# mims-harvard/SubGNN

Measured on AMD Instinct MI355X. Metric: subgraphs/sec fwd+bwd (all 3 channels on) + achieved HBM GB/s, higher is better.
Workload: dtype f32; 1 GPU; synthetic DENSITY-style BA base graph n=1000000 m=10 (9998512 undirected edges), 50000 BFS subgraphs x 20 nodes per GPU (weak form; BASELINE configs[3] "50k sharded across 8" as worded is --scaling strong), all_density hparams (N 10/43, P 57/183, S 42, 1 layer), D=64, full pass = sampling + similarities + fwd + bwd + Adam; subgraphs_per_gpu=50000, subgraphs_total=50000

## Files before the change

include/subgnn_hip.h:

```cpp
#ifndef SUBGNN_HIP_H
#define SUBGNN_HIP_H

#include <stdint.h>

#ifdef __cplusplus
extern "C" {
#endif

#define SGNN_OK                  0
#define SGNN_ERR_BAD_ARG        -1
#define SGNN_ERR_SET_TOO_LARGE  -2
#define SGNN_ERR_NNZ_TOO_LARGE  -3
#define SGNN_ERR_LAUNCH         -4
#define SGNN_ERR_UNSUPPORTED_D  -5

#define SGNN_ABI_VERSION 13
int sgnn_abi_version(void);
int sgnn_warm_up(void* stream);
const char* sgnn_last_error(void);

int sgnn_degree_sequence(const int64_t* rowptr, const int32_t* col, int64_t nnz,
                         const int32_t* full_degree, const uint8_t* self_loops,
                         const int64_t* set_ptr, const int32_t* set_nodes, int64_t n_sets,
                         int64_t max_set_size, int sorted,
                         int32_t* out_internal, int32_t* out_external, const int32_t* set_order, void* stream);
int sgnn_degree_sequence_sorted_rows(const int64_t* rowptr, const int32_t* col, const int32_t* col_sorted,
                                     int64_t nnz, const int32_t* full_degree, const uint8_t* self_loops,
                                     const int64_t* set_ptr, const int32_t* set_nodes, int64_t n_sets,
                                     int64_t max_set_size, int sorted, int32_t* out_internal,
                                     int32_t* out_external, const int32_t* set_order, void* stream);
int sgnn_degree_sequence_hub_bitmaps(const int64_t* rowptr, const int32_t* col, const int32_t* col_sorted,
                                     int64_t nnz, const int32_t* full_degree, const uint8_t* self_loops,
                                     const int32_t* hub_index, const uint32_t* hub_bits, int64_t hub_words,
                                     const int32_t* node_info, int info_degree,
                                     const int64_t* set_ptr, const int32_t* set_nodes, int64_t n_sets,
                                     int64_t max_set_size, int sorted, int32_t* out_internal,
                                     int32_t* out_external, const int32_t* set_order, void* stream);
int64_t sgnn_degree_sequence_search_threshold(void);
int64_t sgnn_degree_sequence_huge_workspace_bytes(int64_t total_entries);
int sgnn_degree_sequence_huge(const int64_t* rowptr, const int32_t* col, int64_t nnz, const int32_t* full_degree,
                              const int64_t* set_ptr, const int32_t* set_nodes, int64_t n_sets,
                              int64_t total_entries, int32_t* out_internal, int32_t* out_external,
                              void* workspace, int64_t workspace_bytes, void* stream);

int sgnn_cc_labels(const int64_t* rowptr, const int32_t* col_sorted, int64_t nnz,
                   const int64_t* sub_ptr, const int32_t* sub_nodes, int64_t n_subgraphs,
                   int64_t max_sub_len ,
                   int32_t* out_label, void* stream);
int sgnn_sort_sets(const int64_t* set_ptr, const int32_t* set_nodes, int64_t n_sets, int64_t max_set_size,
                   int32_t* out_nodes, int32_t* out_pos, void* stream);
int sgnn_cc_compact_stats(const int64_t* sub_ptr, const int32_t* sub_nodes, const int32_t* labels,
                          int64_t n_subgraphs, int64_t max_sub_len, int32_t* out_n_components,
                          int32_t* out_longest, void* stream);
int sgnn_cc_compact(const int64_t* sub_ptr, const int32_t* sub_nodes, const int32_t* labels,
                    int64_t n_subgraphs, int64_t max_sub_len, int64_t C, int64_t L, int64_t* out, void* stream);
int64_t sgnn_cc_huge_workspace_bytes(int64_t total_nodes);
int sgnn_cc_labels_huge(const int64_t* rowptr, const int32_t* col, int64_t nnz, const int64_t* sub_ptr,
                        const int32_t* sub_nodes, int64_t n_subgraphs, int64_t total_nodes, int32_t* out_label,
                        void* workspace, int64_t workspace_bytes, void* stream);
int sgnn_cc_compact_huge(const int64_t* sub_ptr, const int32_t* sub_nodes, const int32_t* labels,
                         int64_t n_subgraphs, int64_t total_nodes, int write, int64_t C, int64_t L,
                         int32_t* out_n_components, int32_t* out_longest, int64_t* out, void* workspace,
                         int64_t workspace_bytes, void* stream);

int64_t sgnn_subgraph_properties_workspace_bytes(int64_t total_nodes);
int sgnn_subgraph_properties(const int64_t* rowptr, const int32_t* col_sorted, int64_t nnz, int64_t max_id, int rows_simple,
                             const int64_t* sub_ptr, const int32_t* sub_nodes, int64_t n_sets, int64_t max_len,
                             int64_t total_nodes, int64_t* out_counts, int32_t* out_core, void* workspace,
                             int64_t workspace_bytes, void* stream);

int64_t sgnn_khop_border_workspace_bytes(int64_t max_id, int64_t n_sets, int bitmap_in_lds);
int sgnn_khop_border_bitmap_fits_lds(int64_t max_id);
int sgnn_khop_border(const int64_t* rowptr, const int32_t* col, int64_t nnz, int64_t max_id,
                     const int64_t* set_ptr, const int32_t* set_nodes, int64_t n_sets,
                     int k, int ego_dict_mode,
                     int64_t* out_count, const int64_t* out_ptr, int32_t* out_nodes, uint8_t* out_hop,
                     void* workspace, int64_t workspace_bytes, int bitmap_in_lds, void* stream);
int sgnn_khop_border_arena(const int64_t* rowptr, const int32_t* col, int64_t nnz, int64_t max_id,
                           const int64_t* set_ptr, const int32_t* set_nodes, int64_t n_sets, int k,
                           const int64_t* arena_off, int32_t* arena, int64_t* out_count,
                           void* workspace, int64_t workspace_bytes, int bitmap_in_lds, void* stream);
int64_t sgnn_khop_border_sample_workspace_bytes(int64_t max_id, int64_t n_sets, int k, int rows_sorted, int bitmap_in_lds);
int sgnn_khop_border_sample(const int64_t* rowptr, const int32_t* col, const int32_t* col_sorted, int64_t nnz, int64_t max_id,
                            const int64_t* set_ptr, const int32_t* set_nodes, int64_t n_sets, int k,
                            int64_t n_slots, uint64_t seed, uint64_t stream_id, int64_t item_base,
                            int64_t* out_anchor, uint8_t* out_hop, uint8_t* out_allneg, int64_t* out_count,
                            const int32_t* set_order ,
                            void* workspace, int64_t workspace_bytes, int bitmap_in_lds, void* stream);
int sgnn_khop_sample_finish(int64_t* anchor, const uint8_t* hop, const uint8_t* allneg, const int64_t* counts,
                            const int64_t* width, int64_t n_sets, int64_t n_slots, float* sims, void* stream);
int sgnn_khop1_border_sorted(const int64_t* rowptr, const int32_t* col, const int32_t* col_sorted, int64_t nnz, int64_t max_id,
                             const int64_t* set_ptr, const int32_t* set_nodes, int64_t n_sets,
                             int64_t* out_count, const int64_t* out_ptr , int32_t* out_ids ,
                             void* workspace, int64_t workspace_bytes, int bitmap_in_lds, void* stream);

int sgnn_first_occurrence_mask(const int64_t* ids, int64_t n_rows, int64_t row_len, uint8_t* keep, void* stream);
int sgnn_filter_sets(const int64_t* set_ptr, const int32_t* set_nodes, const uint8_t* flags, int64_t n_sets, int64_t* counts,
                     const int64_t* out_ptr, int32_t* out_nodes, void* stream);
int sgnn_pack_rows_count(const int64_t* ids, const uint8_t* mask, int64_t n_rows, int64_t row_len, int64_t* counts,
                         void* stream);
int sgnn_pack_rows_write(const int64_t* ids, const uint8_t* mask, int64_t n_rows, int64_t row_len, const int64_t* ptr,
                         int32_t* nodes, void* stream);
int64_t sgnn_pack_fused_max_rows(void);
int64_t sgnn_pack_fused_max_entries(void);
int sgnn_pack_rows_fused(const int64_t* ids, const uint8_t* mask, int mode, int64_t n_rows, int64_t row_len, int64_t* ptr,
                         int32_t* nodes, void* stream);
int sgnn_filter_sets_fused(const int64_t* set_ptr, const int32_t* set_nodes, const uint8_t* flags, int64_t n_sets,
                           int64_t arena_entries, int64_t* out_ptr, int32_t* out_nodes, void* stream);

int sgnn_sample_anchors_padded(const int64_t* ids, int64_t n_rows, int64_t L, int64_t n_slots,
                               uint64_t seed, uint64_t stream_id, int64_t* out, void* stream);
int sgnn_sample_anchors_ragged(const int64_t* set_ptr, const int32_t* set_nodes, int64_t n_sets,
                               const uint8_t* row_has_pad, int64_t n_slots,
                               uint64_t seed, uint64_t stream_id, int64_t item_base, int64_t* out, void* stream);
int sgnn_sample_border_anchors(const int64_t* ptr, const int32_t* ids, const int64_t* counts, int64_t n_sets,
                               const int64_t* width, int64_t n_slots, uint64_t seed, uint64_t stream_id, int64_t item_base,
                               int hop, int64_t* out_anchor, float* out_sims, void* stream);

int sgnn_choice_ragged(const int64_t* ptr, const int32_t* seq, int64_t n_items, int64_t n_draws,
                       uint64_t seed, uint64_t stream_id, int64_t item_base, int64_t* out, void* stream);

int sgnn_set_keys(const int64_t* set_ptr, const int32_t* set_nodes, int64_t n_sets, uint64_t* out_keys, void* stream);
int sgnn_sample_anchors_ragged_keyed(const int64_t* set_ptr, const int32_t* set_nodes, int64_t n_sets,
                                     const uint8_t* row_has_pad, const uint64_t* keys, int64_t n_slots,
                                     uint64_t seed, uint64_t stream_id, int64_t* out, void* stream);
int sgnn_choice_ragged_keyed(const int64_t* ptr, const int32_t* seq, int64_t n_items, const uint64_t* keys, int64_t n_draws,
                             uint64_t seed, uint64_t stream_id, int64_t* out, void* stream);
int sgnn_sample_border_anchors_keyed(const int64_t* ptr, const int32_t* ids, const uint8_t* hops, int64_t n_sets,
                                     const uint8_t* row_has_pad, const uint64_t* keys, int64_t n_slots, uint64_t seed,
                                     uint64_t stream_id, int64_t* out_anchor, float* out_sims, void* stream);

#define SGNN_OCC_NODE 0
#define SGNN_OCC_COMPONENT 1
int64_t sgnn_occlusion_lds_max(void);
int64_t sgnn_occlusion_workspace_bytes(int64_t total_entries);
int sgnn_occlusion_count(const int64_t* set_ptr, const int32_t* set_nodes, int64_t n_sets, int64_t max_set_len, int mode,
                         const int32_t* labels, int64_t* out_units, int64_t* out_variants, int64_t* out_len,
                         int64_t total_entries, void* workspace, int64_t workspace_bytes, void* stream);
int sgnn_occlusion_write(const int64_t* set_ptr, const int32_t* set_nodes, int64_t n_sets, int64_t max_set_len, int mode,
                         const int32_t* labels, const int64_t* var_ptr, const int64_t* len_scan, int64_t n_variants,
                         int64_t* out_ptr, int32_t* out_nodes, int32_t* out_parent, int32_t* out_unit, uint64_t* out_keys,
                         int64_t total_entries, void* workspace, int64_t workspace_bytes, void* stream);

int sgnn_insertion_count(const int64_t* set_ptr, const int32_t* set_nodes, int64_t n_sets, int64_t max_set_len,
                         const int64_t* cand_ptr, const int32_t* cand_ids, int shared, int64_t* out_variants, void* stream);
int sgnn_insertion_write(const int64_t* set_ptr, const int32_t* set_nodes, int64_t n_sets, int64_t max_set_len,
                         const int64_t* cand_ptr, const int32_t* cand_ids, int shared, const int64_t* var_ptr,
                         const int64_t* entry_ptr, int64_t n_variants, int64_t* out_ptr, int32_t* out_nodes,
                         int32_t* out_parent, int32_t* out_cand, uint64_t* out_keys, void* stream);

int64_t sgnn_seeded_walk_max_size(void);
int sgnn_seeded_walk_sets(const int64_t* rowptr, const int32_t* col, int64_t max_id, const int32_t* seeds, int64_t n_seeds,
                          const int32_t* sizes, int64_t per_seed, int64_t width, uint64_t restart_thr, int64_t max_steps,
                          uint64_t seed, uint64_t stream, int64_t item_base, const int64_t* item_ids, int64_t n_items,
                          int32_t* out_nodes, int32_t* out_len, int32_t* out_steps, uint64_t* out_keys, void* stream_handle);

int sgnn_triangular_walks(const int64_t* rowptr, const int32_t* col, const int32_t* col_sorted, int64_t nnz,
                          const int32_t* node_order, int64_t n_nodes,
                          const int64_t* patch_ptr, const int32_t* patch_nodes,
                          const int64_t* inb_ptr, const int32_t* inb_nodes,
                          int mode, int64_t n_items, int64_t walks_per_patch, int64_t walk_len, double beta,
                          uint64_t seed, uint64_t stream_id, int64_t item_base, int64_t max_id, int kernel, int64_t* out,
                          void* stream);
int sgnn_triangular_walks_both(const int64_t* rowptr, const int32_t* col, const int32_t* col_sorted, int64_t nnz,
                               const int64_t* patch_ptr, const int32_t* patch_nodes, const int64_t* inb_ptr,
                               const int32_t* inb_nodes, int64_t n_items, int64_t walks_per_patch, int64_t walk_len,
                               double beta, uint64_t seed, uint64_t stream_id_int, uint64_t stream_id_bor,
                               int64_t item_base, int64_t max_id, int64_t* out, void* stream);
int sgnn_triangular_walks_variants(void);
int sgnn_triangular_walks_rule(int64_t n_walks, int64_t max_id);
int sgnn_triangular_walks_lists(const int64_t* rowptr, const int32_t* col, const int32_t* col_sorted, int64_t nnz,
                                const int32_t* hub_index, const uint32_t* hub_bits, int64_t hub_words,
                                const int32_t* node_order, int64_t n_nodes,
                                const int64_t* patch_ptr, const int32_t* patch_nodes,
                                const int64_t* inb_ptr, const int32_t* inb_nodes,
                                int mode, int64_t n_items, int64_t walks_per_patch, int64_t walk_len, double beta,
                                uint64_t seed, uint64_t stream_id, int64_t item_base, int64_t max_id, int kernel, int variant,
                                int64_t* out, void* stream);
int sgnn_triangular_walks_both_lists(const int64_t* rowptr, const int32_t* col, const int32_t* col_sorted, int64_t nnz,
                                     const int32_t* hub_index, const uint32_t* hub_bits, int64_t hub_words,
                                     const int64_t* patch_ptr, const int32_t* patch_nodes, const int64_t* inb_ptr,
                                     const int32_t* inb_nodes, int64_t n_items, int64_t walks_per_patch, int64_t walk_len,
                                     double beta, uint64_t seed, uint64_t stream_id_int, uint64_t stream_id_bor,
                                     int64_t item_base, int64_t max_id, int variant, int64_t* out, void* stream);

int sgnn_patch_in_border(const int64_t* rowptr, const int32_t* col, int64_t nnz,
                         const int32_t* node_order, const int32_t* node_pos, int64_t n_nodes,
                         const int64_t* patch_ptr, const int32_t* patch_nodes, int64_t n_patches,
                         uint8_t* out_flag, void* stream);
int64_t sgnn_patch_in_border_huge_workspace_bytes(int64_t total_nodes);
int sgnn_patch_in_border_huge(const int64_t* rowptr, const int32_t* col, int64_t nnz,
                              const int32_t* node_order, const int32_t* node_pos, int64_t n_nodes,
                              const int64_t* patch_ptr, const int32_t* patch_nodes, int64_t n_patches,
                              int64_t total_nodes, uint8_t* out_flag, void* workspace, int64_t workspace_bytes,
                              void* stream);

int sgnn_sp_similarity_dense(const double* apsp, int64_t n_cols,
                             const int64_t* set_ptr, const int32_t* set_nodes, int64_t n_sets,
                             float* out, void* stream);
int64_t sgnn_bfs_hops_workspace_bytes(int64_t max_id, int64_t n_sources, int max_hops);
int sgnn_bfs_hops(const int64_t* rowptr, const int32_t* col, int64_t nnz, int64_t max_id,
                  const int32_t* sources, int64_t n_sources, int max_hops, int node_major, int pull_alpha,
                  uint8_t* dist, void* workspace, int64_t workspace_bytes, void* stream);
int sgnn_min_hops_to_sets(const uint8_t* dist, int64_t n_sources, int64_t max_id, int node_major,
                          const int64_t* set_ptr, const int32_t* set_nodes, int64_t n_sets,
                          float* out, void* stream);
int64_t sgnn_bfs_min_hops_workspace_bytes(int64_t max_id, int64_t n_sources, int max_hops, int64_t n_sets);
int sgnn_bfs_min_hops_to_sets(const int64_t* rowptr, const int32_t* col, int64_t nnz, int64_t max_id,
                              const int32_t* sources, int64_t n_sources, int max_hops, int pull_alpha, int push_levels,
                              const int64_t* set_ptr, const int32_t* set_nodes, int64_t n_sets,
                              float* out, int32_t* out_status, void* workspace, int64_t workspace_bytes, void* stream);
int64_t sgnn_graph_component_labels_workspace_bytes(int64_t max_id);
int sgnn_graph_component_labels(const int64_t* rowptr, const int32_t* col, int64_t nnz, int64_t max_id,
                                int32_t* labels, void* workspace, int64_t workspace_bytes, void* stream);
int64_t sgnn_bfs_min_hops_closing_workspace_bytes(int64_t max_id, int64_t n_sources, int max_hops, int64_t n_sets);
int sgnn_bfs_min_hops_to_sets_closing(const int64_t* rowptr, const int32_t* col, int64_t nnz, int64_t max_id,
                                      const int32_t* sources, int64_t n_sources, int max_hops, int pull_alpha, int push_levels,
                                      const int32_t* labels, const int64_t* set_ptr, const int32_t* set_nodes,
                                      int64_t n_sets, float* out, int32_t* out_status, void* workspace, int64_t workspace_bytes,
                                      void* stream);

int sgnn_dtw_order_keys(const int64_t* x_ptr, const int32_t* x_val, int64_t n_x, int64_t* out_keys, void* stream);
int64_t sgnn_dtw_workspace_bytes(int64_t n_x, int64_t max_x_len, int64_t n_y, int64_t max_y_len);
int sgnn_dtw_similarity(const int64_t* x_ptr, const int32_t* x_val, int64_t n_x, int64_t max_x_len,
                        const int64_t* y_ptr, const int32_t* y_val, int64_t n_y, int64_t max_y_len,
                        int tie_order, int kernel, const int32_t* x_order, float* out, void* workspace,
                        int64_t workspace_bytes, void* stream);
int sgnn_dtw_similarity_live(const int64_t* x_ptr, const int32_t* x_val, int64_t n_x, int64_t max_x_len,
                             const int64_t* y_ptr, const int32_t* y_val, int64_t n_y, int64_t max_y_len,
                             int tie_order, int kernel, const int32_t* x_order, const int64_t* x_live_range, float* out,
                             void* workspace, int64_t workspace_bytes, void* stream);
int64_t sgnn_dtw_rows_bytes(int64_t n_x, int64_t max_x_len);
int64_t sgnn_dtw_rows_header_words(void);
int64_t sgnn_dtw_rows_workspace_bytes(int64_t n_x, int64_t max_x_len, int64_t n_y, int64_t max_y_len);
int sgnn_dtw_prepare_rows(const int64_t* x_ptr, const int32_t* x_val, int64_t n_x, int64_t max_x_len, int kernel,
                          const int32_t* x_order, void* rows, int64_t rows_bytes, int64_t* header, void* stream);
int sgnn_dtw_similarity_rows(const int64_t* rows_header, int64_t n_x, int64_t max_x_len,
                             const int64_t* y_ptr, const int32_t* y_val, int64_t n_y, int64_t max_y_len,
                             int tie_order, int kernel, const int32_t* x_order, float* out, void* workspace,
                             int64_t workspace_bytes, void* stream);
int sgnn_dtw_similarity_rows_live(const int64_t* rows_header, int64_t n_x, int64_t max_x_len,
                                  const int64_t* y_ptr, const int32_t* y_val, int64_t n_y, int64_t max_y_len,
                                  int tie_order, int kernel, const int32_t* x_order, const int64_t* x_live_range, float* out,
                                  void* workspace, int64_t workspace_bytes, void* stream);

int64_t sgnn_dtw_exact_workspace_bytes(int64_t n_x, int64_t max_x_len, int64_t n_y, int64_t max_y_len);
int sgnn_dtw_exact_similarity(const int64_t* x_ptr, const int32_t* x_val, int64_t n_x, int64_t max_x_len,
                              const int64_t* y_ptr, const int32_t* y_val, int64_t n_y, int64_t max_y_len,
                              int kernel, const int32_t* x_order, float* out, void* workspace,
                              int64_t workspace_bytes, void* stream);
int sgnn_dtw_exact_similarity_live(const int64_t* x_ptr, const int32_t* x_val, int64_t n_x, int64_t max_x_len,
                                   const int64_t* y_ptr, const int32_t* y_val, int64_t n_y, int64_t max_y_len,
                                   int kernel, const int32_t* x_order, const int64_t* x_live_range, float* out,
                                   void* workspace, int64_t workspace_bytes, void* stream);
int64_t sgnn_dtwx_rows_bytes(int64_t n_x, int64_t max_x_len);
int64_t sgnn_dtwx_rows_workspace_bytes(int64_t n_x, int64_t max_x_len, int64_t n_y, int64_t max_y_len);
int sgnn_dtwx_prepare_rows(const int64_t* x_ptr, const int32_t* x_val, int64_t n_x, int64_t max_x_len, int kernel,
                                const int32_t* x_order, void* rows, int64_t rows_bytes, int64_t* header, void* stream);
int sgnn_dtwx_similarity_rows(const int64_t* rows_header, int64_t n_x, int64_t max_x_len,
                                   const int64_t* y_ptr, const int32_t* y_val, int64_t n_y, int64_t max_y_len,
                                   int kernel, const int32_t* x_order, float* out, void* workspace,
                                   int64_t workspace_bytes, void* stream);
int sgnn_dtwx_similarity_rows_live(const int64_t* rows_header, int64_t n_x, int64_t max_x_len,
                                        const int64_t* y_ptr, const int32_t* y_val, int64_t n_y, int64_t max_y_len,
                                        int kernel, const int32_t* x_order, const int64_t* x_live_range, float* out,
                                        void* workspace, int64_t workspace_bytes, void* stream);

#define SGNN_TOPK_DOT    0
#define SGNN_TOPK_COSINE 1
#define SGNN_TOPK_L2     2
int64_t sgnn_topk_max_k(void);
int64_t sgnn_topk_rows_workspace_bytes(int64_t Q, int64_t N, int64_t k, int64_t splits);
int sgnn_topk_rows(const float* q, int64_t q_stride, int64_t Q, const float* bank, int64_t b_stride, int64_t N,
                   int64_t D, int64_t k, int metric, const float* q_aux, const float* b_aux, const int64_t* exclude,
                   int64_t splits, float* out_score, int64_t* out_index, void* workspace, int64_t workspace_bytes,
                   void* stream);

int64_t sgnn_kmeans_max_k(void);
int64_t sgnn_kmeans_slots(int64_t N, int64_t K, int64_t D);
int64_t sgnn_kmeans_workspace_bytes(int64_t N, int64_t K, int64_t D);
int sgnn_kmeans_step(const float* x, int64_t x_stride, int64_t N, const float* c, int64_t c_stride, int64_t K, int64_t D,
                     int metric, const float* x_aux, const float* c_aux, const int32_t* prev_assign, int32_t* assign,
                     float* score, void* workspace, int64_t workspace_bytes, void* stream);
int sgnn_kmeans_finish(const void* workspace, int64_t workspace_bytes, int64_t N, int64_t K, int64_t D, int metric,
                       const float* c, int64_t c_stride, float* sums, int32_t* counts, double* inertia, int32_t* empty,
                       float* c_next, float* c_aux_next, int32_t* changed, int64_t it, void* stream);

int sgnn_cc_embed_fwd(const float* E, int64_t D,
                      const int64_t* set_ptr, const int32_t* set_nodes, int64_t n_sets,
                      int aggregator, int64_t padded_len, float* out, int32_t* out_arg, void* stream);
int sgnn_cc_embed_fwd_f16(const uint16_t* E_half, int64_t D,
                          const int64_t* set_ptr, const int32_t* set_nodes, int64_t n_sets,
                          int aggregator, int64_t padded_len, float* out, int32_t* out_arg, void* stream);
int sgnn_cc_embed_bwd(const float* grad_out, int64_t D,
                      const int64_t* set_ptr, const int32_t* set_nodes, int64_t n_sets,
                      int aggregator, const int32_t* arg, float* grad_E, void* stream);

#define SGNN_SRC_DENSE  0
#define SGNN_SRC_GATHER 1
#define SGNN_SRC_SHARED 2

typedef struct sgnn_mpn_args {
    int32_t src;
    int32_t sims_per_edge;
    int64_t R, A, D;
    const float*   x;
    const int64_t* ids;
    int64_t        id_div;
    const uint8_t* edge_mask;
    const uint8_t* row_mask;
    const float*   sims;
    int64_t        sims_ld;
    const int64_t* sim_col;
    const float*   wp;
    const float*   bp;
    int32_t        x_f16;
    const float*   z_act;
    int32_t        flags;
} sgnn_mpn_args;
#define SGNN_MPN_WP_PARTIAL 1
#define SGNN_MPN_RELU_Z     2

int sgnn_mpn_fwd_chunks(const sgnn_mpn_args* args);
int sgnn_mpn_fwd(const sgnn_mpn_args* args, float* agg , float* z , void* stream);
int64_t sgnn_mpn_fwd_many_max_bodies(void);
int sgnn_mpn_fwd_many(int64_t n, const sgnn_mpn_args* args, float* const* agg, float* const* z, void* stream);
int sgnn_mpn_bwd(const sgnn_mpn_args* args, const float* grad_agg, const float* grad_z,
                 float* grad_x, float* grad_wp, void* stream);

int sgnn_attn_scores_epilogue(const float* XU, const float* qW, const float* v, int64_t R, int64_t H,
                              int64_t rows_per_batch, float* out, void* stream);
int64_t sgnn_attn_scores_f16_workspace_bytes(int64_t H);
int sgnn_attn_scores_fwd_f16(const float* X, const float* U, const float* qW, const float* v,
                             int64_t R, int64_t H, int64_t rows_per_batch, float* out,
                             void* workspace, int64_t workspace_bytes, void* stream);

int sgnn_lstm_supported(int64_t hidden_size);
int sgnn_lstm_fwd(const float* pre_x, const float* whh_f, const float* whh_r, const float* bhh_f, const float* bhh_r,
                  int64_t B, int64_t T, int64_t hidden_size, float* y, float* gates, float* cell, float* hprev, void* stream);
int sgnn_lstm_bwd(const float* whh_f, const float* whh_r, const float* gates, const float* cell, const float* dy,
                  int64_t B, int64_t T, int64_t hidden_size, float* dgates, void* stream);

int sgnn_rows_gemm(const float* X, const int64_t* ids, int64_t ldx, int64_t R, int64_t K, const float* W0, const float* W1,
                   const float* b0, const float* b1, int64_t N, float* out, float* x_copy, void* stream);
int sgnn_rows_gemm_nt(const float* A, int64_t R, int64_t K, const float* W0, const float* W1, int64_t N, float* out, void* stream);
int sgnn_lstm_tail_fwd(const float* y, int64_t n_patches, int64_t n_walks, int64_t T, int64_t H2, int last_only,
                       const float* W_lin, const float* b_lin, int64_t D, float* s_out, float* X, void* stream);
int sgnn_lstm_tail_bwd(const float* dX, const float* s, int64_t n_patches, int64_t n_walks, int64_t T, int64_t H2,
                       int last_only, const float* W_lin, int64_t D, float* dy, float* dW_lin, float* db_lin, void* stream);

int sgnn_masked_sum_slot_fwd(const float* x, const uint8_t* mask, int64_t B, int64_t C, int64_t W, float* out,
                             int64_t out_ld, void* stream);
int sgnn_masked_sum_slot_bwd(const float* grad_out, int64_t grad_ld, const uint8_t* mask, int64_t B, int64_t C,
                             int64_t W, float* grad_x, void* stream);
int sgnn_masked_sum_slots_fwd(const float* const* xs, const int64_t* widths, const int64_t* offsets, int64_t n_pieces,
                              const uint8_t* mask, int64_t B, int64_t C, float* out, int64_t out_ld, void* stream);
int sgnn_masked_sum_slots_bwd(const float* grad_out, int64_t grad_ld, const uint8_t* mask, int64_t B, int64_t C,
                              float* const* grad_xs, const int64_t* widths, const int64_t* offsets, int64_t n_pieces, void* stream);

int64_t sgnn_cross_entropy_workspace_bytes(int64_t B);
int sgnn_cross_entropy_fwd(const float* logits, const int64_t* labels, int64_t B, int64_t K, float* lse, float* loss,
                           float* accuracy, void* workspace, int64_t workspace_bytes, void* stream);
int sgnn_cross_entropy_bwd(const float* logits, const int64_t* labels, const float* lse, const float* grad_loss,
                           int64_t B, int64_t K, float* grad_logits, void* stream);

int64_t sgnn_bce_logits_workspace_bytes(int64_t B);
int sgnn_bce_logits_fwd(const float* logits, const int64_t* targets, int64_t B, int64_t K, float* loss, float* accuracy,
                        void* workspace, int64_t workspace_bytes, void* stream);
int sgnn_bce_logits_bwd(const float* logits, const int64_t* targets, const float* grad_loss, int64_t B, int64_t K,
                        float* grad_logits, void* stream);

int sgnn_cross_entropy_fwd_weighted(const float* logits, const int64_t* labels, int64_t B, int64_t K, float* lse, float* loss,
                                    float* accuracy, void* workspace, int64_t workspace_bytes, void* stream,
                                    const float* class_weight);
int sgnn_cross_entropy_bwd_weighted(const float* logits, const int64_t* labels, const float* lse, const float* grad_loss,
                                    int64_t B, int64_t K, float* grad_logits, void* stream, const float* class_weight);
int sgnn_bce_logits_fwd_weighted(const float* logits, const int64_t* targets, int64_t B, int64_t K, float* loss, float* accuracy,
                                 void* workspace, int64_t workspace_bytes, void* stream, const float* weight,
                                 const float* pos_weight);
int sgnn_bce_logits_bwd_weighted(const float* logits, const int64_t* targets, const float* grad_loss, int64_t B, int64_t K,
                                 float* grad_logits, void* stream, const float* weight, const float* pos_weight);

int64_t sgnn_column_sum_workspace_bytes(int64_t R, int64_t A);
int sgnn_column_sum(const float* x, int64_t ld, int64_t R, int64_t A, float* out, void* workspace, int64_t workspace_bytes,
                    void* stream);

int64_t sgnn_readout_many_max(void);
int sgnn_readout_many_fwd(int64_t n, const float* const* sims, const int64_t* sims_ld, const int64_t* const* sim_col,
                          const float* const* X, const float* const* wp, const float* const* bp,
                          const int64_t* const* ids, const uint8_t* const* row_mask, float* const* s, const int64_t* A,
                          const int64_t* off, int64_t D, int64_t B, int64_t C, float* out, int64_t out_ld, void* stream);
int64_t sgnn_readout_many_bwd_workspace_bytes(int64_t n, const int64_t* A, int64_t B, int64_t C);
int sgnn_readout_many_bwd(int64_t n, const float* grad_out, int64_t grad_ld, const float* const* sims, const int64_t* sims_ld,
                          const int64_t* const* sim_col, const float* const* X, const float* const* wp,
                          const float* const* bp, const int64_t* const* ids, const uint8_t* const* row_mask,
                          float* const* s, const int64_t* A, const int64_t* off, int64_t D, int64_t B, int64_t C,
                          float* const* grad_X, float* const* grad_wp, float* const* grad_bp, void* workspace,
                          int64_t workspace_bytes, unsigned* tickets, void* stream);

int64_t sgnn_scatter_add_rows_workspace_bytes(int64_t n_edges, int64_t D);
int64_t sgnn_sort_edges_by_key_workspace_bytes(int64_t n_edges, int64_t max_key);
int sgnn_sort_edges_by_key(const int32_t* keys, int64_t n_edges, int64_t max_key, int32_t* key_sorted, int32_t* order,
                           void* workspace, int64_t workspace_bytes, void* stream);
int sgnn_scatter_add_rows_sorted(const int32_t* order, const int32_t* key_sorted, int64_t n_edges,
                                 const int32_t* edge_row, int64_t edges_per_row,
                                 const float* G, int64_t D, const float* c1, const float* c2, const float* v,
                                 const int32_t* arg, float* table,
                                 void* workspace, int64_t workspace_bytes, void* stream);
int64_t sgnn_scatter_add_rows_multi_workspace_bytes(int64_t total_edges, int64_t D, int64_t max_key);
int sgnn_scatter_add_rows_multi(int64_t n_lists, const int32_t* const* keys, const int64_t* n_edges,
                                const int32_t* const* edge_row, const int64_t* edges_per_row, const float* const* G,
                                const float* const* c1, const float* const* c2, const float* const* v, int64_t D,
                                int64_t max_key, float* table, void* workspace, int64_t workspace_bytes, void* stream);
int64_t sgnn_mpn_bwd_shared_det_workspace_bytes(int64_t R, int64_t A, int64_t D);
int sgnn_mpn_bwd_shared_det(const struct sgnn_mpn_args* args, const float* grad_agg, const float* grad_z,
                            float* grad_x, float* grad_wp, float* grad_bp, void* workspace, int64_t workspace_bytes,
                            void* stream);
int sgnn_mpn_bwd_edges(const struct sgnn_mpn_args* args, const float* grad_z, int32_t* out_keys, float* out_c1,
                       float* out_c2, void* stream);
int sgnn_mpn_bwd_wp_partial(const struct sgnn_mpn_args* args, const float* grad_z, float* partial, int64_t partial_ld,
                            void* stream);
int sgnn_mpn_bwd_edges_many(int64_t n, const struct sgnn_mpn_args* args, const float* const* grad_z, int32_t* const* out_keys,
                            float* const* out_c1, float* const* out_c2, void* stream);

int sgnn_update_fwd(const float* x, const float* aggr, const float* W, const float* b, int64_t R, int64_t D,
                    float* out, void* stream);
int64_t sgnn_update_fwd_chunks_max_rows(void);
int sgnn_update_fwd_chunks(const float* x, const float* aggr_chunks, int64_t n_chunks, const float* W, const float* b,
                           int64_t R, int64_t D, float* out, float* aggr_sum, void* stream);
int64_t sgnn_update_many_max_bodies(void);
int sgnn_update_fwd_many(int64_t n, const float* const* x, const float* const* aggr_chunks, const int64_t* n_chunks,
                         const float* const* W, const float* const* b, int64_t R, int64_t D, float* const* out,
                         float* const* aggr_sum, void* stream);
int sgnn_update_bwd_many(int64_t n, const float* const* grad_out, const float* const* out, const float* const* x,
                         const float* const* aggr, const float* const* W, int64_t R, int64_t D, float* const* grad_x,
                         float* const* grad_aggr, float* const* grad_W, float* const* grad_b, void* workspace,
                         int64_t workspace_bytes, void* stream);
int64_t sgnn_update_bwd_workspace_bytes(int64_t R, int64_t D);
int sgnn_update_bwd(const float* grad_out, const float* out, const float* x, const float* aggr, const float* W,
                    int64_t R, int64_t D, float* grad_x, float* grad_aggr, float* grad_W, float* grad_b,
                    void* workspace, int64_t workspace_bytes, void* stream);

int sgnn_adam_step(float* param, const float* grad, float* exp_avg, float* exp_avg_sq, int64_t n, float lr, float beta1,
                   float beta2, float eps, float weight_decay, int64_t step, const float* grad_scale, void* stream);

int64_t sgnn_optim_partials(const int64_t* numels, int64_t n_tensors);
int sgnn_optim_sumsq(const float* const* grads, const int64_t* numels, int64_t n_tensors, float* partial,
                     int64_t* step_counters, const int64_t* counter_slots, void* stream);
int sgnn_optim_count(int64_t* step_counters, const int64_t* counter_slots, int64_t n_tensors, void* stream);
int sgnn_optim_adam(float* const* params, float* const* grads, float* const* exp_avg, float* const* exp_avg_sq,
                    const int64_t* numels, const int32_t* zero_grad, int64_t n_tensors, float lr, float beta1, float beta2,
                    float eps, const int64_t* steps, const int64_t* step_counters, const int64_t* counter_slots,
                    const int64_t* row_lens, unsigned char* const* row_seen,
                    const float* partial, int64_t n_partial, float max_norm, float* coef_out, void* stream);
int sgnn_optim_adam_lr_table(float* const* params, float* const* grads, float* const* exp_avg, float* const* exp_avg_sq,
                             const int64_t* numels, const int32_t* zero_grad, int64_t n_tensors, const float* lr_table,
                             int64_t lr_len, float beta1, float beta2, float eps, const int64_t* steps,
                             const int64_t* step_counters, const int64_t* counter_slots, const int64_t* row_lens,
                             unsigned char* const* row_seen, const float* partial, int64_t n_partial, float max_norm,
                             float* coef_out, void* stream);


int64_t sgnn_gather_rows_many_max(void);
int sgnn_gather_rows_many(int64_t n, const void* const* src, void* const* dst, const int64_t* row_bytes,
                          const int64_t* src_rows, const int64_t* idx, int64_t B, int32_t* out_of_range, void* stream);

int sgnn_head_supported(int64_t H1, int64_t H2, int64_t K);
int64_t sgnn_head_blocks(int64_t B);
int64_t sgnn_head_partial_floats(int64_t H1, int64_t H2, int64_t K);
int64_t sgnn_head_fwd_workspace_bytes(int64_t B);
int sgnn_head_fwd(const float* z1, int64_t B, int64_t H1, int64_t H2, int64_t K, const float* W2, const float* b2,
                  const float* W3, const float* b3, const int64_t* labels, float p, int64_t* rng, float* a1, float* a2,
                  float* logits, float* lse, float* out, void* workspace, int64_t workspace_bytes, void* stream);
int sgnn_head_bwd(const float* logits, const float* lse, const int64_t* labels, const float* grad_loss,
                  const float* grad_logits, const float* rows, const float* a1, const float* a2, const float* W2,
                  const float* W3, int64_t B, int64_t H1, int64_t H2, int64_t K, float p, float* dz1, float* partial,
                  void* stream);

int sgnn_head_fwd_ml(const float* z1, int64_t B, int64_t H1, int64_t H2, int64_t K, const float* W2, const float* b2,
                     const float* W3, const float* b3, const int64_t* targets, float p, int64_t* rng, float* a1, float* a2,
                     float* logits, float* out, void* workspace, int64_t workspace_bytes, void* stream);
int sgnn_head_bwd_ml(const float* logits, const int64_t* targets, const float* grad_loss, const float* grad_logits,
                     const float* rows, const float* a1, const float* a2, const float* W2, const float* W3, int64_t B,
                     int64_t H1, int64_t H2, int64_t K, float p, float* dz1, float* partial, void* stream);

int sgnn_head_fwd_weighted(const float* z1, int64_t B, int64_t H1, int64_t H2, int64_t K, const float* W2, const float* b2,
                           const float* W3, const float* b3, const int64_t* labels, float p, int64_t* rng, float* a1, float* a2,
                           float* logits, float* lse, float* out, void* workspace, int64_t workspace_bytes, void* stream,
                           const float* class_weight);
int sgnn_head_bwd_weighted(const float* logits, const float* lse, const int64_t* labels, const float* grad_loss,
                           const float* grad_logits, const float* rows, const float* a1, const float* a2, const float* W2,
                           const float* W3, int64_t B, int64_t H1, int64_t H2, int64_t K, float p, float* dz1, float* partial,
                           void* stream, const float* class_weight);
int sgnn_head_fwd_ml_weighted(const float* z1, int64_t B, int64_t H1, int64_t H2, int64_t K, const float* W2, const float* b2,
                              const float* W3, const float* b3, const int64_t* targets, float p, int64_t* rng, float* a1,
                              float* a2, float* logits, float* out, void* workspace, int64_t workspace_bytes, void* stream,
                              const float* weight, const float* pos_weight);
int sgnn_head_bwd_ml_weighted(const float* logits, const int64_t* targets, const float* grad_loss, const float* grad_logits,
                              const float* rows, const float* a1, const float* a2, const float* W2, const float* W3, int64_t B,
                              int64_t H1, int64_t H2, int64_t K, float p, float* dz1, float* partial, void* stream,
                              const float* weight, const float* pos_weight);

int64_t sgnn_contract_rows_max_jobs(void);
int64_t sgnn_contract_rows_blocks(int64_t R, int64_t M, int64_t N);
int sgnn_contract_rows_partial(int64_t n_jobs, const float* const* A, const float* const* B, const int64_t* lda,
                               const int64_t* ldb, const int64_t* M, const int64_t* N, const int64_t* R,
                               float* const* part, float* const* colsum_part, void* stream);
int64_t sgnn_reduce_partials_max_jobs(void);
int sgnn_reduce_partials(int64_t n_jobs, const float* const* part, const int64_t* n_blocks, const int64_t* n,
                         float* const* out, void* stream);

int64_t sgnn_ne_chunk_entries(void);
int sgnn_ne_aggregate(const int64_t* rowptr, const int32_t* col, const float* w, const float* a_self, const float* X,
                      const float* bias, int64_t n_rows, int64_t F, const int32_t* chunk_row, const int64_t* chunk_beg,
                      int64_t n_chunks, const int32_t* long_rows, const int64_t* chunk_first, int64_t n_long,
                      int relu, uint32_t drop_thr, float drop_scale, uint64_t seed, uint64_t stream_id, float* out,
                      float* partial, void* stream);
int sgnn_ne_relu_drop_bwd(const float* grad, const float* out, float* dst, int64_t n, float scale, void* stream);
int sgnn_ne_negatives(const int64_t* rowptr, const int32_t* col_sorted, int64_t n_ids, int64_t n, uint64_t seed,
                      uint64_t stream_id, int64_t item_base, int max_attempts, int32_t* u_out, int32_t* v_out, void* stream);
int64_t sgnn_ne_link_loss_workspace_bytes(void);
int sgnn_ne_link_loss(const float* Z, int64_t F, const int32_t* pu, const int32_t* pv, int64_t n_pairs, int64_t n_pos,
                      float* s_out, float* g_out, float* loss, void* workspace, int64_t workspace_bytes, void* stream);

int sgnn_probe_stream_copy(const void* src, void* dst, int64_t n_bytes, int bytes_per_lane, void* stream);

#ifdef __cplusplus
}
#endif
#endif
```

subgnn_amd/_lib.py:

```python
import ctypes
import os

_HERE = os.path.dirname(os.path.abspath(__file__))
LIB_PATH = os.path.join(_HERE, 'lib', 'libsubgnn_hip.so')

c_i64 = ctypes.c_int64
c_u64 = ctypes.c_uint64
c_int = ctypes.c_int
c_dbl = ctypes.c_double
c_ptr = ctypes.c_void_p


class MpnArgs(ctypes.Structure):
    _fields_ = [('src', ctypes.c_int32), ('sims_per_edge', ctypes.c_int32),
                ('R', c_i64), ('A', c_i64), ('D', c_i64),
                ('x', c_ptr), ('ids', c_ptr), ('id_div', c_i64), ('edge_mask', c_ptr), ('row_mask', c_ptr),
                ('sims', c_ptr), ('sims_ld', c_i64), ('sim_col', c_ptr), ('wp', c_ptr), ('bp', c_ptr),
                ('x_f16', ctypes.c_int32), ('z_act', c_ptr), ('flags', ctypes.c_int32)]


SIGNATURES = {
    'sgnn_abi_version': (c_int, []),
    'sgnn_warm_up': (c_int, [c_ptr]),
    'sgnn_last_error': (ctypes.c_char_p, []),
    'sgnn_degree_sequence': (c_int, [c_ptr, c_ptr, c_i64, c_ptr, c_ptr, c_ptr, c_ptr, c_i64, c_i64, c_int, c_ptr, c_ptr,
                                     c_ptr, c_ptr]),
    'sgnn_degree_sequence_sorted_rows': (c_int, [c_ptr, c_ptr, c_ptr, c_i64, c_ptr, c_ptr, c_ptr, c_ptr, c_i64, c_i64, c_int,
                                                 c_ptr, c_ptr, c_ptr, c_ptr]),
    'sgnn_degree_sequence_hub_bitmaps': (c_int, [c_ptr, c_ptr, c_ptr, c_i64, c_ptr, c_ptr, c_ptr, c_ptr, c_i64, c_ptr, c_int,
                                                 c_ptr, c_ptr, c_i64, c_i64, c_int, c_ptr, c_ptr, c_ptr, c_ptr]),
    'sgnn_degree_sequence_search_threshold': (c_i64, []),
    'sgnn_cc_embed_fwd_f16': (c_int, [c_ptr, c_i64, c_ptr, c_ptr, c_i64, c_int, c_i64, c_ptr, c_ptr, c_ptr]),
    'sgnn_cc_labels': (c_int, [c_ptr, c_ptr, c_i64, c_ptr, c_ptr, c_i64, c_i64, c_ptr, c_ptr]),
    'sgnn_cc_compact_stats': (c_int, [c_ptr, c_ptr, c_ptr, c_i64, c_i64, c_ptr, c_ptr, c_ptr]),
    'sgnn_cc_compact': (c_int, [c_ptr, c_ptr, c_ptr, c_i64, c_i64, c_i64, c_i64, c_ptr, c_ptr]),
    'sgnn_cc_huge_workspace_bytes': (c_i64, [c_i64]),
    'sgnn_degree_sequence_huge_workspace_bytes': (c_i64, [c_i64]),
    'sgnn_degree_sequence_huge': (c_int, [c_ptr, c_ptr, c_i64, c_ptr, c_ptr, c_ptr, c_i64, c_i64, c_ptr, c_ptr, c_ptr, c_i64, c_ptr]),
    'sgnn_cc_labels_huge': (c_int, [c_ptr, c_ptr, c_i64, c_ptr, c_ptr, c_i64, c_i64, c_ptr, c_ptr, c_i64, c_ptr]),
    'sgnn_cc_compact_huge': (c_int, [c_ptr, c_ptr, c_ptr, c_i64, c_i64, c_int, c_i64, c_i64, c_ptr, c_ptr, c_ptr, c_ptr, c_i64, c_ptr]),
    'sgnn_subgraph_properties_workspace_bytes': (c_i64, [c_i64]),
    'sgnn_subgraph_properties': (c_int, [c_ptr, c_ptr, c_i64, c_i64, c_int, c_ptr, c_ptr, c_i64, c_i64, c_i64, c_ptr, c_ptr, c_ptr, c_i64,
                                         c_ptr]),
    'sgnn_patch_in_border_huge_workspace_bytes': (c_i64, [c_i64]),
    'sgnn_patch_in_border_huge': (c_int, [c_ptr, c_ptr, c_i64, c_ptr, c_ptr, c_i64, c_ptr, c_ptr, c_i64, c_i64, c_ptr, c_ptr, c_i64, c_ptr]),
    'sgnn_sort_sets': (c_int, [c_ptr, c_ptr, c_i64, c_i64, c_ptr, c_ptr, c_ptr]),
    'sgnn_khop_border_workspace_bytes': (c_i64, [c_i64, c_i64, c_int]),
    'sgnn_khop_border_bitmap_fits_lds': (c_int, [c_i64]),
    'sgnn_khop_border': (c_int, [c_ptr, c_ptr, c_i64, c_i64, c_ptr, c_ptr, c_i64, c_int, c_int, c_ptr, c_ptr, c_ptr,
                                 c_ptr, c_ptr, c_i64, c_int, c_ptr]),
    'sgnn_khop_border_arena': (c_int, [c_ptr, c_ptr, c_i64, c_i64, c_ptr, c_ptr, c_i64, c_int, c_ptr, c_ptr, c_ptr, c_ptr,
                                       c_i64, c_int, c_ptr]),
    'sgnn_khop_border_sample_workspace_bytes': (c_i64, [c_i64, c_i64, c_int, c_int, c_int]),
    'sgnn_khop_border_sample': (c_int, [c_ptr, c_ptr, c_ptr, c_i64, c_i64, c_ptr, c_ptr, c_i64, c_int, c_i64, c_u64, c_u64, c_i64,
                                        c_ptr, c_ptr, c_ptr, c_ptr, c_ptr, c_ptr, c_i64, c_int, c_ptr]),
    'sgnn_khop1_border_sorted': (c_int, [c_ptr, c_ptr, c_ptr, c_i64, c_i64, c_ptr, c_ptr, c_i64, c_ptr, c_ptr, c_ptr, c_ptr, c_i64,
                                         c_int, c_ptr]),
    'sgnn_sample_border_anchors': (c_int, [c_ptr, c_ptr, c_ptr, c_i64, c_ptr, c_i64, c_u64, c_u64, c_i64, c_int, c_ptr, c_ptr,
                                           c_ptr]),
    'sgnn_sample_anchors_padded': (c_int, [c_ptr, c_i64, c_i64, c_i64, c_u64, c_u64, c_ptr, c_ptr]),
    'sgnn_sample_anchors_ragged': (c_int, [c_ptr, c_ptr, c_i64, c_ptr, c_i64, c_u64, c_u64, c_i64, c_ptr, c_ptr]),
    'sgnn_choice_ragged': (c_int, [c_ptr, c_ptr, c_i64, c_i64, c_u64, c_u64, c_i64, c_ptr, c_ptr]),
    'sgnn_set_keys': (c_int, [c_ptr, c_ptr, c_i64, c_ptr, c_ptr]),
    'sgnn_occlusion_lds_max': (c_i64, []),
    'sgnn_occlusion_workspace_bytes': (c_i64, [c_i64]),
    'sgnn_occlusion_count': (c_int, [c_ptr, c_ptr, c_i64, c_i64, c_int, c_ptr, c_ptr, c_ptr, c_ptr, c_i64, c_ptr, c_i64, c_ptr]),
    'sgnn_occlusion_write': (c_int, [c_ptr, c_ptr, c_i64, c_i64, c_int, c_ptr, c_ptr, c_ptr, c_i64, c_ptr, c_ptr, c_ptr, c_ptr, c_ptr,
                                     c_i64, c_ptr, c_i64, c_ptr]),
    'sgnn_insertion_count': (c_int, [c_ptr, c_ptr, c_i64, c_i64, c_ptr, c_ptr, c_int, c_ptr, c_ptr]),
    'sgnn_insertion_write': (c_int, [c_ptr, c_ptr, c_i64, c_i64, c_ptr, c_ptr, c_int, c_ptr, c_ptr, c_i64, c_ptr, c_ptr, c_ptr, c_ptr,
                                     c_ptr, c_ptr]),
    'sgnn_seeded_walk_max_size': (c_i64, []),
    'sgnn_seeded_walk_sets': (c_int, [c_ptr, c_ptr, c_i64, c_ptr, c_i64, c_ptr, c_i64, c_i64, c_u64, c_i64, c_u64, c_u64, c_i64,
                                      c_ptr, c_i64, c_ptr, c_ptr, c_ptr, c_ptr, c_ptr]),
    'sgnn_sample_anchors_ragged_keyed': (c_int, [c_ptr, c_ptr, c_i64, c_ptr, c_ptr, c_i64, c_u64, c_u64, c_ptr, c_ptr]),
    'sgnn_choice_ragged_keyed': (c_int, [c_ptr, c_ptr, c_i64, c_ptr, c_i64, c_u64, c_u64, c_ptr, c_ptr]),
    'sgnn_sample_border_anchors_keyed': (c_int, [c_ptr, c_ptr, c_ptr, c_i64, c_ptr, c_ptr, c_i64, c_u64, c_u64, c_ptr, c_ptr,
                                                 c_ptr]),
    'sgnn_triangular_walks_both': (c_int, [c_ptr, c_ptr, c_ptr, c_i64, c_ptr, c_ptr, c_ptr, c_ptr, c_i64, c_i64, c_i64, c_dbl, c_u64,
                                           c_u64, c_u64, c_i64, c_i64, c_ptr, c_ptr]),
    'sgnn_triangular_walks': (c_int, [c_ptr, c_ptr, c_ptr, c_i64, c_ptr, c_i64, c_ptr, c_ptr, c_ptr, c_ptr, c_int,
                                      c_i64, c_i64, c_i64, c_dbl, c_u64, c_u64, c_i64, c_i64, c_int, c_ptr, c_ptr]),
    'sgnn_triangular_walks_variants': (c_int, []),
    'sgnn_triangular_walks_rule': (c_int, [c_i64, c_i64]),
    'sgnn_triangular_walks_lists': (c_int, [c_ptr, c_ptr, c_ptr, c_i64, c_ptr, c_ptr, c_i64, c_ptr, c_i64, c_ptr, c_ptr, c_ptr, c_ptr,
                                            c_int, c_i64, c_i64, c_i64, c_dbl, c_u64, c_u64, c_i64, c_i64, c_int, c_int, c_ptr, c_ptr]),
    'sgnn_triangular_walks_both_lists': (c_int, [c_ptr, c_ptr, c_ptr, c_i64, c_ptr, c_ptr, c_i64, c_ptr, c_ptr, c_ptr, c_ptr, c_i64,
                                                 c_i64, c_i64, c_dbl, c_u64, c_u64, c_u64, c_i64, c_i64, c_int, c_ptr, c_ptr]),
    'sgnn_patch_in_border': (c_int, [c_ptr, c_ptr, c_i64, c_ptr, c_ptr, c_i64, c_ptr, c_ptr, c_i64, c_ptr, c_ptr]),
    'sgnn_sp_similarity_dense': (c_int, [c_ptr, c_i64, c_ptr, c_ptr, c_i64, c_ptr, c_ptr]),
    'sgnn_bfs_hops_workspace_bytes': (c_i64, [c_i64, c_i64, c_int]),
    'sgnn_bfs_min_hops_workspace_bytes': (c_i64, [c_i64, c_i64, c_int, c_i64]),
    'sgnn_bfs_min_hops_to_sets': (c_int, [c_ptr, c_ptr, c_i64, c_i64, c_ptr, c_i64, c_int, c_int, c_int, c_ptr, c_ptr, c_i64, c_ptr, c_ptr,
                                          c_ptr, c_i64, c_ptr]),
    'sgnn_graph_component_labels_workspace_bytes': (c_i64, [c_i64]),
    'sgnn_graph_component_labels': (c_int, [c_ptr, c_ptr, c_i64, c_i64, c_ptr, c_ptr, c_i64, c_ptr]),
    'sgnn_bfs_min_hops_closing_workspace_bytes': (c_i64, [c_i64, c_i64, c_int, c_i64]),
    'sgnn_bfs_min_hops_to_sets_closing': (c_int, [c_ptr, c_ptr, c_i64, c_i64, c_ptr, c_i64, c_int, c_int, c_int, c_ptr, c_ptr,
                                                  c_ptr, c_i64, c_ptr, c_ptr, c_ptr, c_i64, c_ptr]),
    'sgnn_bfs_hops': (c_int, [c_ptr, c_ptr, c_i64, c_i64, c_ptr, c_i64, c_int, c_int, c_int, c_ptr, c_ptr, c_i64, c_ptr]),
    'sgnn_min_hops_to_sets': (c_int, [c_ptr, c_i64, c_i64, c_int, c_ptr, c_ptr, c_i64, c_ptr, c_ptr]),
    'sgnn_dtw_workspace_bytes': (c_i64, [c_i64, c_i64, c_i64, c_i64]),
    'sgnn_dtw_similarity': (c_int, [c_ptr, c_ptr, c_i64, c_i64, c_ptr, c_ptr, c_i64, c_i64, c_int, c_int, c_ptr, c_ptr, c_ptr,
                                    c_i64, c_ptr]),
    'sgnn_dtw_order_keys': (c_int, [c_ptr, c_ptr, c_i64, c_ptr, c_ptr]),
    'sgnn_dtw_similarity_live': (c_int, [c_ptr, c_ptr, c_i64, c_i64, c_ptr, c_ptr, c_i64, c_i64, c_int, c_int, c_ptr, c_ptr, c_ptr,
                                         c_ptr, c_i64, c_ptr]),
    'sgnn_dtw_rows_bytes': (c_i64, [c_i64, c_i64]),
    'sgnn_dtw_rows_header_words': (c_i64, []),
    'sgnn_dtw_rows_workspace_bytes': (c_i64, [c_i64, c_i64, c_i64, c_i64]),
    'sgnn_dtw_prepare_rows': (c_int, [c_ptr, c_ptr, c_i64, c_i64, c_int, c_ptr, c_ptr, c_i64, c_ptr, c_ptr]),
    'sgnn_dtw_similarity_rows': (c_int, [c_ptr, c_i64, c_i64, c_ptr, c_ptr, c_i64, c_i64, c_int, c_int, c_ptr, c_ptr, c_ptr,
                                         c_i64, c_ptr]),
    'sgnn_dtw_similarity_rows_live': (c_int, [c_ptr, c_i64, c_i64, c_ptr, c_ptr, c_i64, c_i64, c_int, c_int, c_ptr, c_ptr, c_ptr,
                                              c_ptr, c_i64, c_ptr]),
    'sgnn_dtwx_rows_bytes': (c_i64, [c_i64, c_i64]),
    'sgnn_dtwx_rows_workspace_bytes': (c_i64, [c_i64, c_i64, c_i64, c_i64]),
    'sgnn_dtwx_prepare_rows': (c_int, [c_ptr, c_ptr, c_i64, c_i64, c_int, c_ptr, c_ptr, c_i64, c_ptr, c_ptr]),
    'sgnn_dtwx_similarity_rows': (c_int, [c_ptr, c_i64, c_i64, c_ptr, c_ptr, c_i64, c_i64, c_int, c_ptr, c_ptr, c_ptr,
                                               c_i64, c_ptr]),
    'sgnn_dtwx_similarity_rows_live': (c_int, [c_ptr, c_i64, c_i64, c_ptr, c_ptr, c_i64, c_i64, c_int, c_ptr, c_ptr, c_ptr,
                                                    c_ptr, c_i64, c_ptr]),
    'sgnn_topk_max_k': (c_i64, []),
    'sgnn_topk_rows_workspace_bytes': (c_i64, [c_i64, c_i64, c_i64, c_i64]),
    'sgnn_topk_rows': (c_int, [c_ptr, c_i64, c_i64, c_ptr, c_i64, c_i64, c_i64, c_i64, c_int, c_ptr, c_ptr, c_ptr, c_i64, c_ptr,
                               c_ptr, c_ptr, c_i64, c_ptr]),
    'sgnn_kmeans_max_k': (c_i64, []),
    'sgnn_kmeans_slots': (c_i64, [c_i64, c_i64, c_i64]),
    'sgnn_kmeans_workspace_bytes': (c_i64, [c_i64, c_i64, c_i64]),
    'sgnn_kmeans_step': (c_int, [c_ptr, c_i64, c_i64, c_ptr, c_i64, c_i64, c_i64, c_int, c_ptr, c_ptr, c_ptr, c_ptr, c_ptr, c_ptr,
                                 c_i64, c_ptr]),
    'sgnn_kmeans_finish': (c_int, [c_ptr, c_i64, c_i64, c_i64, c_i64, c_int, c_ptr, c_i64, c_ptr, c_ptr, c_ptr, c_ptr, c_ptr, c_ptr,
                                   c_ptr, c_i64, c_ptr]),
    'sgnn_dtw_exact_workspace_bytes': (c_i64, [c_i64, c_i64, c_i64, c_i64]),
    'sgnn_dtw_exact_similarity': (c_int, [c_ptr, c_ptr, c_i64, c_i64, c_ptr, c_ptr, c_i64, c_i64, c_int, c_ptr, c_ptr, c_ptr,
                                          c_i64, c_ptr]),
    'sgnn_dtw_exact_similarity_live': (c_int, [c_ptr, c_ptr, c_i64, c_i64, c_ptr, c_ptr, c_i64, c_i64, c_int, c_ptr, c_ptr, c_ptr,
                                               c_ptr, c_i64, c_ptr]),
    'sgnn_cc_embed_fwd': (c_int, [c_ptr, c_i64, c_ptr, c_ptr, c_i64, c_int, c_i64, c_ptr, c_ptr, c_ptr]),
    'sgnn_cc_embed_bwd': (c_int, [c_ptr, c_i64, c_ptr, c_ptr, c_i64, c_int, c_ptr, c_ptr, c_ptr]),
    'sgnn_mpn_fwd_chunks': (c_int, [ctypes.POINTER(MpnArgs)]),
    'sgnn_mpn_fwd': (c_int, [ctypes.POINTER(MpnArgs), c_ptr, c_ptr, c_ptr]),
    'sgnn_mpn_fwd_many_max_bodies': (c_i64, []),
    'sgnn_mpn_fwd_many': (c_int, [c_i64, c_ptr, c_ptr, c_ptr, c_ptr]),
    'sgnn_mpn_bwd': (c_int, [ctypes.POINTER(MpnArgs), c_ptr, c_ptr, c_ptr, c_ptr, c_ptr]),
    'sgnn_attn_scores_epilogue': (c_int, [c_ptr, c_ptr, c_ptr, c_i64, c_i64, c_i64, c_ptr, c_ptr]),
    'sgnn_attn_scores_f16_workspace_bytes': (c_i64, [c_i64]),
    'sgnn_attn_scores_fwd_f16': (c_int, [c_ptr, c_ptr, c_ptr, c_ptr, c_i64, c_i64, c_i64, c_ptr, c_ptr, c_i64, c_ptr]),
    'sgnn_lstm_supported': (c_int, [c_i64]),
    'sgnn_lstm_fwd': (c_int, [c_ptr, c_ptr, c_ptr, c_ptr, c_ptr, c_i64, c_i64, c_i64, c_ptr, c_ptr, c_ptr, c_ptr, c_ptr]),
    'sgnn_lstm_bwd': (c_int, [c_ptr, c_ptr, c_ptr, c_ptr, c_ptr, c_i64, c_i64, c_i64, c_ptr, c_ptr]),
    'sgnn_masked_sum_slot_fwd': (c_int, [c_ptr, c_ptr, c_i64, c_i64, c_i64, c_ptr, c_i64, c_ptr]),
    'sgnn_masked_sum_slot_bwd': (c_int, [c_ptr, c_i64, c_ptr, c_i64, c_i64, c_i64, c_ptr, c_ptr]),
    'sgnn_masked_sum_slots_fwd': (c_int, [c_ptr, c_ptr, c_ptr, c_i64, c_ptr, c_i64, c_i64, c_ptr, c_i64, c_ptr]),
    'sgnn_masked_sum_slots_bwd': (c_int, [c_ptr, c_i64, c_ptr, c_i64, c_i64, c_ptr, c_ptr, c_ptr, c_i64, c_ptr]),
    'sgnn_first_occurrence_mask': (c_int, [c_ptr, c_i64, c_i64, c_ptr, c_ptr]),
    'sgnn_filter_sets': (c_int, [c_ptr, c_ptr, c_ptr, c_i64, c_ptr, c_ptr, c_ptr, c_ptr]),
    'sgnn_pack_rows_count': (c_int, [c_ptr, c_ptr, c_i64, c_i64, c_ptr, c_ptr]),
    'sgnn_pack_rows_write': (c_int, [c_ptr, c_ptr, c_i64, c_i64, c_ptr, c_ptr, c_ptr]),
    'sgnn_pack_fused_max_rows': (c_i64, []),
    'sgnn_pack_fused_max_entries': (c_i64, []),
    'sgnn_pack_rows_fused': (c_int, [c_ptr, c_ptr, c_int, c_i64, c_i64, c_ptr, c_ptr, c_ptr]),
    'sgnn_filter_sets_fused': (c_int, [c_ptr, c_ptr, c_ptr, c_i64, c_i64, c_ptr, c_ptr, c_ptr]),
    'sgnn_khop_sample_finish': (c_int, [c_ptr, c_ptr, c_ptr, c_ptr, c_ptr, c_i64, c_i64, c_ptr, c_ptr]),
    'sgnn_cross_entropy_workspace_bytes': (c_i64, [c_i64]),
    'sgnn_cross_entropy_fwd': (c_int, [c_ptr, c_ptr, c_i64, c_i64, c_ptr, c_ptr, c_ptr, c_ptr, c_i64, c_ptr]),
    'sgnn_cross_entropy_bwd': (c_int, [c_ptr, c_ptr, c_ptr, c_ptr, c_i64, c_i64, c_ptr, c_ptr]),
    'sgnn_bce_logits_workspace_bytes': (c_i64, [c_i64]),
    'sgnn_bce_logits_fwd': (c_int, [c_ptr, c_ptr, c_i64, c_i64, c_ptr, c_ptr, c_ptr, c_i64, c_ptr]),
    'sgnn_bce_logits_bwd': (c_int, [c_ptr, c_ptr, c_ptr, c_i64, c_i64, c_ptr, c_ptr]),
    'sgnn_cross_entropy_fwd_weighted': (c_int, [c_ptr, c_ptr, c_i64, c_i64, c_ptr, c_ptr, c_ptr, c_ptr, c_i64, c_ptr, c_ptr]),
    'sgnn_cross_entropy_bwd_weighted': (c_int, [c_ptr, c_ptr, c_ptr, c_ptr, c_i64, c_i64, c_ptr, c_ptr, c_ptr]),
    'sgnn_bce_logits_fwd_weighted': (c_int, [c_ptr, c_ptr, c_i64, c_i64, c_ptr, c_ptr, c_ptr, c_i64, c_ptr, c_ptr, c_ptr]),
    'sgnn_bce_logits_bwd_weighted': (c_int, [c_ptr, c_ptr, c_ptr, c_i64, c_i64, c_ptr, c_ptr, c_ptr, c_ptr]),
    'sgnn_column_sum_workspace_bytes': (c_i64, [c_i64, c_i64]),
    'sgnn_column_sum': (c_int, [c_ptr, c_i64, c_i64, c_i64, c_ptr, c_ptr, c_i64, c_ptr]),
    'sgnn_gather_rows_many_max': (c_i64, []),
    'sgnn_rows_gemm': (c_int, [c_ptr, c_ptr, c_i64, c_i64, c_i64, c_ptr, c_ptr, c_ptr, c_ptr, c_i64, c_ptr, c_ptr, c_ptr]),
    'sgnn_rows_gemm_nt': (c_int, [c_ptr, c_i64, c_i64, c_ptr, c_ptr, c_i64, c_ptr, c_ptr]),
    'sgnn_lstm_tail_fwd': (c_int, [c_ptr, c_i64, c_i64, c_i64, c_i64, c_int, c_ptr, c_ptr, c_i64, c_ptr, c_ptr, c_ptr]),
    'sgnn_lstm_tail_bwd': (c_int, [c_ptr, c_ptr, c_i64, c_i64, c_i64, c_i64, c_int, c_ptr, c_i64, c_ptr, c_ptr, c_ptr, c_ptr]),
    'sgnn_readout_many_max': (c_i64, []),
    'sgnn_readout_many_fwd': (c_int, [c_i64, c_ptr, c_ptr, c_ptr, c_ptr, c_ptr, c_ptr, c_ptr, c_ptr, c_ptr, c_ptr, c_ptr, c_i64, c_i64,
                                      c_i64, c_ptr, c_i64, c_ptr]),
    'sgnn_readout_many_bwd_workspace_bytes': (c_i64, [c_i64, c_ptr, c_i64, c_i64]),
    'sgnn_readout_many_bwd': (c_int, [c_i64, c_ptr, c_i64, c_ptr, c_ptr, c_ptr, c_ptr, c_ptr, c_ptr, c_ptr, c_ptr, c_ptr, c_ptr, c_ptr,
                                      c_i64, c_i64, c_i64, c_ptr, c_ptr, c_ptr, c_ptr, c_i64, c_ptr, c_ptr]),
    'sgnn_gather_rows_many': (c_int, [c_i64, c_ptr, c_ptr, c_ptr, c_ptr, c_ptr, c_i64, c_ptr, c_ptr]),
    'sgnn_head_supported': (c_int, [c_i64, c_i64, c_i64]),
    'sgnn_head_blocks': (c_i64, [c_i64]),
    'sgnn_head_partial_floats': (c_i64, [c_i64, c_i64, c_i64]),
    'sgnn_head_fwd_workspace_bytes': (c_i64, [c_i64]),
    'sgnn_head_fwd': (c_int, [c_ptr, c_i64, c_i64, c_i64, c_i64, c_ptr, c_ptr, c_ptr, c_ptr, c_ptr, ctypes.c_float, c_ptr, c_ptr, c_ptr,
                              c_ptr, c_ptr, c_ptr, c_ptr, c_i64, c_ptr]),
    'sgnn_head_bwd': (c_int, [c_ptr, c_ptr, c_ptr, c_ptr, c_ptr, c_ptr, c_ptr, c_ptr, c_ptr, c_ptr, c_i64, c_i64, c_i64, c_i64,
                              ctypes.c_float, c_ptr, c_ptr, c_ptr]),
    'sgnn_head_fwd_ml': (c_int, [c_ptr, c_i64, c_i64, c_i64, c_i64, c_ptr, c_ptr, c_ptr, c_ptr, c_ptr, ctypes.c_float, c_ptr, c_ptr, c_ptr,
                                 c_ptr, c_ptr, c_ptr, c_i64, c_ptr]),
    'sgnn_head_bwd_ml': (c_int, [c_ptr, c_ptr, c_ptr, c_ptr, c_ptr, c_ptr, c_ptr, c_ptr, c_ptr, c_i64, c_i64, c_i64, c_i64,
                                 ctypes.c_float, c_ptr, c_ptr, c_ptr]),
    'sgnn_head_fwd_weighted': (c_int, [c_ptr, c_i64, c_i64, c_i64, c_i64, c_ptr, c_ptr, c_ptr, c_ptr, c_ptr, ctypes.c_float, c_ptr, c_ptr,
                                       c_ptr, c_ptr, c_ptr, c_ptr, c_ptr, c_i64, c_ptr, c_ptr]),
    'sgnn_head_bwd_weighted': (c_int, [c_ptr, c_ptr, c_ptr, c_ptr, c_ptr, c_ptr, c_ptr, c_ptr, c_ptr, c_ptr, c_i64, c_i64, c_i64, c_i64,
                                       ctypes.c_float, c_ptr, c_ptr, c_ptr, c_ptr]),
    'sgnn_head_fwd_ml_weighted': (c_int, [c_ptr, c_i64, c_i64, c_i64, c_i64, c_ptr, c_ptr, c_ptr, c_ptr, c_ptr, ctypes.c_float, c_ptr, c_ptr,
                                          c_ptr, c_ptr, c_ptr, c_ptr, c_i64, c_ptr, c_ptr, c_ptr]),
    'sgnn_head_bwd_ml_weighted': (c_int, [c_ptr, c_ptr, c_ptr, c_ptr, c_ptr, c_ptr, c_ptr, c_ptr, c_ptr, c_i64, c_i64, c_i64, c_i64,
                                          ctypes.c_float, c_ptr, c_ptr, c_ptr, c_ptr, c_ptr]),
    'sgnn_contract_rows_max_jobs': (c_i64, []),
    'sgnn_contract_rows_blocks': (c_i64, [c_i64, c_i64, c_i64]),
    'sgnn_contract_rows_partial': (c_int, [c_i64, c_ptr, c_ptr, c_ptr, c_ptr, c_ptr, c_ptr, c_ptr, c_ptr, c_ptr, c_ptr]),
    'sgnn_reduce_partials_max_jobs': (c_i64, []),
    'sgnn_reduce_partials': (c_int, [c_i64, c_ptr, c_ptr, c_ptr, c_ptr, c_ptr]),
    'sgnn_probe_stream_copy': (c_int, [c_ptr, c_ptr, c_i64, c_int, c_ptr]),
    'sgnn_scatter_add_rows_workspace_bytes': (c_i64, [c_i64, c_i64]),
    'sgnn_mpn_bwd_shared_det_workspace_bytes': (c_i64, [c_i64, c_i64, c_i64]),
    'sgnn_mpn_bwd_shared_det': (c_int, [c_ptr, c_ptr, c_ptr, c_ptr, c_ptr, c_ptr, c_ptr, c_i64, c_ptr]),
    'sgnn_adam_step': (c_int, [c_ptr, c_ptr, c_ptr, c_ptr, c_i64, ctypes.c_float, ctypes.c_float, ctypes.c_float, ctypes.c_float,
                               ctypes.c_float, c_i64, c_ptr, c_ptr]),
    'sgnn_optim_partials': (c_i64, [c_ptr, c_i64]),
    'sgnn_optim_sumsq': (c_int, [c_ptr, c_ptr, c_i64, c_ptr, c_ptr, c_ptr, c_ptr]),
    'sgnn_optim_count': (c_int, [c_ptr, c_ptr, c_i64, c_ptr]),
    'sgnn_optim_adam': (c_int, [c_ptr, c_ptr, c_ptr, c_ptr, c_ptr, c_ptr, c_i64, ctypes.c_float, ctypes.c_float, ctypes.c_float,
                                ctypes.c_float, c_ptr, c_ptr, c_ptr, c_ptr, c_ptr, c_ptr, c_i64, ctypes.c_float, c_ptr, c_ptr]),
    'sgnn_optim_adam_lr_table': (c_int, [c_ptr, c_ptr, c_ptr, c_ptr, c_ptr, c_ptr, c_i64, c_ptr, c_i64, ctypes.c_float,
                                         ctypes.c_float, ctypes.c_float, c_ptr, c_ptr, c_ptr, c_ptr, c_ptr, c_ptr, c_i64,
                                         ctypes.c_float, c_ptr, c_ptr]),
    'sgnn_update_fwd': (c_int, [c_ptr, c_ptr, c_ptr, c_ptr, c_i64, c_i64, c_ptr, c_ptr]),
    'sgnn_update_fwd_chunks_max_rows': (c_i64, []),
    'sgnn_update_fwd_chunks': (c_int, [c_ptr, c_ptr, c_i64, c_ptr, c_ptr, c_i64, c_i64, c_ptr, c_ptr, c_ptr]),
    'sgnn_update_many_max_bodies': (c_i64, []),
    'sgnn_update_fwd_many': (c_int, [c_i64, c_ptr, c_ptr, c_ptr, c_ptr, c_ptr, c_i64, c_i64, c_ptr, c_ptr, c_ptr]),
    'sgnn_update_bwd_many': (c_int, [c_i64, c_ptr, c_ptr, c_ptr, c_ptr, c_ptr, c_i64, c_i64, c_ptr, c_ptr, c_ptr, c_ptr, c_ptr, c_i64,
                                     c_ptr]),
    'sgnn_update_bwd_workspace_bytes': (c_i64, [c_i64, c_i64]),
    'sgnn_update_bwd': (c_int, [c_ptr, c_ptr, c_ptr, c_ptr, c_ptr, c_i64, c_i64, c_ptr, c_ptr, c_ptr, c_ptr, c_ptr, c_i64, c_ptr]),
    'sgnn_sort_edges_by_key_workspace_bytes': (c_i64, [c_i64, c_i64]),
    'sgnn_sort_edges_by_key': (c_int, [c_ptr, c_i64, c_i64, c_ptr, c_ptr, c_ptr, c_i64, c_ptr]),
    'sgnn_scatter_add_rows_sorted': (c_int, [c_ptr, c_ptr, c_i64, c_ptr, c_i64, c_ptr, c_i64, c_ptr, c_ptr, c_ptr, c_ptr, c_ptr,
                                             c_ptr, c_i64, c_ptr]),
    'sgnn_scatter_add_rows_multi_workspace_bytes': (c_i64, [c_i64, c_i64, c_i64]),
    'sgnn_scatter_add_rows_multi': (c_int, [c_i64, c_ptr, c_ptr, c_ptr, c_ptr, c_ptr, c_ptr, c_ptr, c_ptr, c_i64, c_i64, c_ptr, c_ptr,
                                            c_i64, c_ptr]),
    'sgnn_mpn_bwd_edges': (c_int, [ctypes.POINTER(MpnArgs), c_ptr, c_ptr, c_ptr, c_ptr, c_ptr]),
    'sgnn_mpn_bwd_edges_many': (c_int, [c_i64, c_ptr, c_ptr, c_ptr, c_ptr, c_ptr, c_ptr]),
    'sgnn_mpn_bwd_wp_partial': (c_int, [ctypes.POINTER(MpnArgs), c_ptr, c_ptr, c_i64, c_ptr]),
    'sgnn_ne_chunk_entries': (c_i64, []),
    'sgnn_ne_aggregate': (c_int, [c_ptr, c_ptr, c_ptr, c_ptr, c_ptr, c_ptr, c_i64, c_i64, c_ptr, c_ptr, c_i64, c_ptr, c_ptr, c_i64,
                                  c_int, ctypes.c_uint32, ctypes.c_float, c_u64, c_u64, c_ptr, c_ptr, c_ptr]),
    'sgnn_ne_relu_drop_bwd': (c_int, [c_ptr, c_ptr, c_ptr, c_i64, ctypes.c_float, c_ptr]),
    'sgnn_ne_negatives': (c_int, [c_ptr, c_ptr, c_i64, c_i64, c_u64, c_u64, c_i64, c_int, c_ptr, c_ptr, c_ptr]),
    'sgnn_ne_link_loss_workspace_bytes': (c_i64, []),
    'sgnn_ne_link_loss': (c_int, [c_ptr, c_i64, c_ptr, c_ptr, c_i64, c_i64, c_ptr, c_ptr, c_ptr, c_ptr, c_i64, c_ptr]),
}

ERRORS = {-1: 'SGNN_ERR_BAD_ARG', -2: 'SGNN_ERR_SET_TOO_LARGE', -3: 'SGNN_ERR_NNZ_TOO_LARGE',
          -4: 'SGNN_ERR_LAUNCH', -5: 'SGNN_ERR_UNSUPPORTED_D'}

_lib = None


class SubgnnHipError(RuntimeError):
    pass


def load():
    global _lib
    if _lib is not None:
        return _lib
    import torch
    if not os.path.exists(LIB_PATH):
        raise SubgnnHipError('libsubgnn_hip.so is missing (%s): build it with `python -m subgnn_amd.build`; '
                             'this package has no CPU fallback' % LIB_PATH)
    lib = ctypes.CDLL(LIB_PATH)
    for name, (res, args) in SIGNATURES.items():
        fn = getattr(lib, name)
        fn.restype = res
        fn.argtypes = args
    if lib.sgnn_abi_version() != 13:
        raise SubgnnHipError('ABI version mismatch')
    _lib = lib
    return lib


def check(rc, what):
    if rc != 0:
        lib = load()
        detail = lib.sgnn_last_error().decode() if rc == -4 else ''
        raise SubgnnHipError('%s failed: %s %s' % (what, ERRORS.get(rc, rc), detail))
```

subgnn_amd/build.py:

```python
import os
import subprocess
import sys

HERE = os.path.dirname(os.path.abspath(__file__))
CSRC = os.path.join(HERE, 'csrc')
LIBDIR = os.path.join(HERE, 'lib')
LIB = os.path.join(LIBDIR, 'libsubgnn_hip.so')
SOURCES = ['lib.hip', 'degree_sequence.hip', 'graph_sets.hip', 'samplers.hip', 'similarity.hip', 'dtw.hip', 'dtw_exact.hip', 'embed.hip', 'mpn.hip', 'attention.hip', 'lstm.hip', 'probe.hip', 'scatter.hip', 'update.hip', 'optim.hip', 'readout.hip', 'loss.hip', 'head.hip', 'node_emb.hip', 'subgraph_props.hip', 'neighbors.hip', 'occlusion.hip', 'insertion.hip', 'seeded_sets.hip', 'kmeans.hip']
ARCH = 'gfx950'
EXTRA_FLAGS = {'dtw.hip': ['-fno-honor-nans', '-mllvm', '-disable-promote-alloca-to-vector'],
               'dtw_exact.hip': ['-fno-honor-nans', '-mllvm', '-disable-promote-alloca-to-vector']}
HEADERS = [os.path.join(CSRC, 'common.h'), os.path.join(CSRC, 'dtw_cost.h'), os.path.join(CSRC, 'id_table.h'), os.path.join(CSRC, 'topk_order.h'), os.path.join(HERE, '..', 'include', 'subgnn_hip.h')]


def _hipcc():
    for c in (os.environ.get('HIPCC'), '/opt/rocm/bin/hipcc', 'hipcc'):
        if c and (os.path.isabs(c) and os.path.exists(c) or not os.path.isabs(c)):
            return c
    raise RuntimeError('hipcc not found')


def needs_build():
    if not os.path.exists(LIB):
        return True
    t = os.path.getmtime(LIB)
    deps = [os.path.join(CSRC, s) for s in SOURCES] + HEADERS
    return any(os.path.getmtime(d) > t for d in deps)


def build(force=False, verbose=True):
    if not force and not needs_build():
        return LIB
    os.makedirs(LIBDIR, exist_ok=True)
    objs = []
    for s in SOURCES:
        o = os.path.join(LIBDIR, s.replace('.hip', '.o'))
        src = os.path.join(CSRC, s)
        if force or not os.path.exists(o) or os.path.getmtime(o) < max(os.path.getmtime(f) for f in [src] + HEADERS):
            cmd = [_hipcc(), '--offload-arch=' + ARCH, '-O3', '-fPIC', '-std=c++17', '-munsafe-fp-atomics',
                   '-Wall', '-Wno-unused-function'] + EXTRA_FLAGS.get(s, []) + os.environ.get('SGNN_HIPCC_FLAGS', '').split() + ['-c', src, '-o', o]
            if verbose:
                print(' '.join(cmd), flush=True)
            subprocess.check_call(cmd)
        objs.append(o)
    cmd = [_hipcc(), '--offload-arch=' + ARCH, '-shared', '-fPIC', '-o', LIB] + objs
    if verbose:
        print(' '.join(cmd), flush=True)
    subprocess.check_call(cmd)
    return LIB


if __name__ == '__main__':
    build(force='--force' in sys.argv)
    print(LIB)
```

subgnn_amd/csrc/dtw.hip:

```cpp
#include "common.h"
#include "dtw_cost.h"
#include <type_traits>
#include <cstdlib>

#define DTW_THREADS 256
#ifndef DTW_BLOCKS
#define DTW_BLOCKS (256 * 2)
#endif
#define DTW_NT ((int64_t)DTW_THREADS * DTW_BLOCKS)
#ifndef DTW_REG_BLOCKS
#define DTW_REG_BLOCKS (256 * 32)
#endif
#define DTW_REG_NT ((int64_t)DTW_THREADS * DTW_REG_BLOCKS)
#define DTW_MAX_LEVELS 16

struct DtwLayout {
    int64_t MX, MY;
    int64_t XL, YL;
    int64_t n_dbl;
    int64_t n_i32;
    int64_t n_dir;
    int64_t xoff[DTW_MAX_LEVELS], yoff[DTW_MAX_LEVELS];
};

static inline DtwLayout dtw_layout(int64_t MX, int64_t MY) {
    DtwLayout L;
    L.MX = MX; L.MY = MY;
    int64_t xo = 0, yo = 0;
    for (int k = 0; k < DTW_MAX_LEVELS; ++k) {
        L.xoff[k] = xo; L.yoff[k] = yo;
        xo += (MX >> k) > 0 ? (MX >> k) : 0;
        yo += (MY >> k) > 0 ? (MY >> k) : 0;
    }
    L.XL = xo; L.YL = yo;
    L.n_dbl = 2 * MY;
    L.n_i32 = 4 * MX;
    L.n_dir = (MX * MY + 15) / 16;
    return L;
}

static inline int64_t dtw_align8(int64_t b) { return (b + 7) / 8 * 8; }

static inline bool dtw_words_in_lds(int64_t max_y_len) { return (max_y_len >> 1) * DTW_THREADS * 4 <= 48 * 1024; }
static inline int64_t dtw_scratch_bytes(const DtwLayout& L) {
    const int64_t lane = L.n_dbl * 8 + dtw_align8(L.n_i32 * 4) + dtw_align8(L.n_dir * 4);
    int64_t scratch = DTW_NT * lane;
    const int64_t reg = dtw_words_in_lds(L.MY) ? 0 : dtw_align8(DTW_REG_NT * (L.YL - L.MY) * 4);
    return reg > scratch ? reg : scratch;
}

extern "C" int64_t sgnn_dtw_workspace_bytes(int64_t n_x, int64_t max_x_len, int64_t n_y, int64_t max_y_len) {
    if (max_x_len < 1) max_x_len = 1;
    if (max_y_len < 1) max_y_len = 1;
    const DtwLayout L = dtw_layout(max_x_len, max_y_len);
    return dtw_scratch_bytes(L)
         + 2 * (n_x * L.XL * 8 + n_y * L.YL * 8) + dtw_align8(n_x * 4) + dtw_align8(n_y * 4);
}

__global__ void dtw_pyramid_kernel(const int64_t* __restrict__ ptr, const int32_t* __restrict__ val, int64_t n,
                                   int64_t M, int64_t PL, int transposed, double* __restrict__ out,
                                   double* __restrict__ rec, int32_t* __restrict__ len_out,
                                   const int32_t* __restrict__ order)
{
    for (int64_t s = blockIdx.x * (int64_t)blockDim.x + threadIdx.x; s < n; s += (int64_t)gridDim.x * blockDim.x) {
        const int64_t src = order ? order[s] : s;
        const int64_t b = ptr[src];
        int len = (int)(ptr[src + 1] - b);
        len_out[s] = len;
#define PYI(e) (transposed ? (int64_t)(e) * n + s : s * PL + (e))
#define PY(e) out[PYI(e)]
        for (int i = 0; i < len; ++i) { const double v = (double)val[b + i]; PY(i) = v; rec[PYI(i)] = 1.0 / (v + 1.0); }
        int64_t off = 0;
        int k = 0;
        while (len >= 2 && k + 1 < DTW_MAX_LEVELS) {
            const int64_t noff = off + (M >> k);
            const int nlen = len / 2;
            for (int i = 0; i < nlen; ++i) {
                const double v = (PY(off + 2 * i) + PY(off + 2 * i + 1)) / 2.0;
                PY(noff + i) = v;
                rec[PYI(noff + i)] = 1.0 / (v + 1.0);
            }
            off = noff; len = nlen; ++k;
        }
#undef PY
#undef PYI
    }
}

__global__ __launch_bounds__(256) void dtw_pyramid_wave_kernel(const int64_t* __restrict__ ptr, const int32_t* __restrict__ val,
                                                               int64_t n, int64_t M, int64_t PL, int transposed,
                                                               double* __restrict__ out, double* __restrict__ rec,
                                                               int32_t* __restrict__ len_out, const int32_t* __restrict__ order)
{
    extern __shared__ double pyr_sh[];
    const int lane = threadIdx.x & 63, wave = threadIdx.x >> 6;
    const int64_t s = blockIdx.x * 4ll + wave;
    if (s >= n) return;
    double* buf = pyr_sh + (int64_t)wave * 2 * M;
    const int64_t src = order ? order[s] : s;
    const int64_t b = ptr[src];
    int len = (int)(ptr[src + 1] - b);
    if (lane == 0) len_out[s] = len;
#define PYI(e) (transposed ? (int64_t)(e) * n + s : s * PL + (e))
    for (int i = lane; i < len; i += 64) {
        const double v = (double)val[b + i];
        buf[i] = v;
        out[PYI(i)] = v;
        rec[PYI(i)] = 1.0 / (v + 1.0);
    }
    int64_t off = 0;
    int k = 0;
    while (len >= 2 && k + 1 < DTW_MAX_LEVELS) {
        __builtin_amdgcn_fence(__ATOMIC_RELEASE, "wavefront");
        __builtin_amdgcn_wave_barrier();
        __builtin_amdgcn_fence(__ATOMIC_ACQUIRE, "wavefront");
        const int64_t noff = off + (M >> k);
        const int nlen = len / 2;
        for (int i = lane; i < nlen; i += 64) {
            const double v = (buf[off + 2 * i] + buf[off + 2 * i + 1]) / 2.0;
            buf[noff + i] = v;
            out[PYI(noff + i)] = v;
            rec[PYI(noff + i)] = 1.0 / (v + 1.0);
        }
        off = noff; len = nlen; ++k;
    }
#undef PYI
}

#define DTW_PYR_WAVE_MAX_SERIES 8192
#define DTW_PYR_WAVE_MAX_LEN 1024

static void dtw_launch_pyramid(const int64_t* ptr, const int32_t* val, int64_t n, int64_t M, int64_t PL, int transposed,
                               double* out, double* rec, int32_t* len_out, const int32_t* order, hipStream_t st)
{
    if (n <= DTW_PYR_WAVE_MAX_SERIES && M <= DTW_PYR_WAVE_MAX_LEN)
        hipLaunchKernelGGL(dtw_pyramid_wave_kernel, dim3((unsigned)((n + 3) / 4)), dim3(256), (size_t)(4 * 2 * M * sizeof(double)), st,
                           ptr, val, n, M, PL, transposed, out, rec, len_out, order);
    else
        hipLaunchKernelGGL(dtw_pyramid_kernel, dim3(sgnn_grid_for(n, 256)), dim3(256), 0, st, ptr, val, n, M, PL, transposed, out,
                           rec, len_out, order);
}

__device__ __forceinline__ double dtw_mask_cost(bool in, double dt) {
    return __hiloint2double(in ? __double2hiint(dt) : 0x7fe00000, __double2loint(dt));
}

__global__ __launch_bounds__(DTW_THREADS) void dtw_similarity_kernel(
    const double* __restrict__ xpyr, const int32_t* __restrict__ xlen, int64_t n_x,
    const double* __restrict__ ypyr, const int32_t* __restrict__ ylen, int64_t n_y,
    int tie_order, float* __restrict__ out, double* __restrict__ wd, int32_t* __restrict__ wi,
    uint32_t* __restrict__ wb, DtwLayout L)
{
    const int64_t NT = (int64_t)gridDim.x * blockDim.x;
    const int64_t tid = blockIdx.x * (int64_t)blockDim.x + threadIdx.x;
#define WD(k) wd[(int64_t)(k) * NT + tid]
#define WI(k) wi[(int64_t)(k) * NT + tid]
#define WB(k) wb[(int64_t)(k) * NT + tid]
#define ROWSTART(i) WI(i)
#define LOHI(i) WI(L.MX + (i))
#define FL(h, i) WI((2 + (h)) * L.MX + (i))
    const int o0 = tie_order == 0 ? 0 : 2, o1 = tie_order == 0 ? 1 : 0, o2 = tie_order == 0 ? 2 : 1;
    const double INF = __longlong_as_double(0x7ff0000000000000ll);
    const int64_t total = n_x * n_y;
    for (int64_t pair = tid; pair < total; pair += NT) {
        const int64_t a = pair / n_x, r = pair % n_x;
        const int lx0 = xlen[r], ly0 = ylen[a];
        if (lx0 == 0 || ly0 == 0) { out[r * n_y + a] = 0.f; continue; }
        const double* __restrict__ yp = ypyr + a * L.YL;
        int n_levels = 1;
        {
            int lx = lx0, ly = ly0;
            while (lx >= 3 && ly >= 3) { lx >>= 1; ly >>= 1; ++n_levels; }
        }
        double result = 0.0;
        for (int lev = n_levels - 1; lev >= 0; --lev) {
            const int lx = lx0 >> lev, ly = ly0 >> lev;
            const int64_t xo = L.xoff[lev], yo = L.yoff[lev];
            const int hc = lev & 1, hp = (lev + 1) & 1;
            if (lev == n_levels - 1) {
                int cells = 0;
                for (int i = 0; i < lx; ++i) { LOHI(i) = (ly - 1) << 16; ROWSTART(i) = cells; cells += ly; }
            } else {
                const int lxc = lx0 >> (lev + 1);
                int prev_lo = 0, cells = 0;
                for (int i = 0; i < lx; ++i) {
                    const int ci = i >> 1;
                    const int ca = ci - 1 < 0 ? 0 : (ci - 1 > lxc - 1 ? lxc - 1 : ci - 1);
                    const int cb = ci + 1 > lxc - 1 ? lxc - 1 : ci + 1;
                    int lo = 2 * ((FL(hp, ca) & 0xffff) - 1);
                    int hi = 2 * ((FL(hp, cb) >> 16) + 1) + 1;
                    if (lo < prev_lo) lo = prev_lo;
                    if (lo < 0) lo = 0;
                    if (hi > ly - 1) hi = ly - 1;
                    if (hi < lo) { lo = 1; hi = 0; }
                    LOHI(i) = (hi << 16) | lo;
                    ROWSTART(i) = cells;
                    if (hi >= lo) { cells += hi - lo + 1; prev_lo = lo; }
                }
            }
            int64_t prow = 0, crow = L.MY;
            int plo = 0, phi = -1;
            uint32_t acc = 0;
            int cell = 0;
            for (int i = 0; i < lx; ++i) {
                const int lohi = LOHI(i);
                const int lo = lohi & 0xffff, hi = lohi >> 16;
                const double xi = xpyr[(xo + i) * n_x + r];
                double left = INF;
                double diag = INF;
                if (i == 0) { if (lo == 0) diag = 0.0; }
                else if (lo - 1 >= plo && lo - 1 <= phi) diag = WD(prow + lo - 1);
                for (int j = lo; j <= hi; ++j) {
                    const double dt = dtw_cost(xi, yp[yo + j]);
                    double up = INF;
                    if (i > 0 && j >= plo && j <= phi) up = WD(prow + j);
                    double c[3];
                    c[0] = up + dt; c[1] = left + dt; c[2] = diag + dt;
                    int best = o0;
                    double bc = c[o0];
                    if (tie_order == 2) {
                        best = (diag <= up && diag <= left) ? 2 : (up <= left ? 0 : 1);
                        bc = c[best];
                    } else {
                        if (c[o1] < bc) { bc = c[o1]; best = o1; }
                        if (c[o2] < bc) { bc = c[o2]; best = o2; }
                    }
                    WD(crow + j) = bc;
                    acc |= (uint32_t)best << ((cell & 15) * 2);
                    if ((cell & 15) == 15) { WB(cell >> 4) = acc; acc = 0; }
                    ++cell;
                    left = bc;
                    diag = up;
                }
                if (hi >= lo) { const int64_t t = prow; prow = crow; crow = t; plo = lo; phi = hi; }
            }
            if (cell & 15) WB(cell >> 4) = acc;
            result = WD(prow + (ly - 1));
            if (lev == 0) break;
            for (int q = 0; q < lx; ++q) FL(hc, q) = (int32_t)((0xffffu << 16) | 0xffffu);
            int i = lx - 1, j = ly - 1;
            while (i >= 0 && j >= 0) {
                const int fl = FL(hc, i);
                int first = fl & 0xffff, last = fl >> 16;
                if (last < j) last = j;
                if (first > j) first = j;
                FL(hc, i) = (last << 16) | first;
                const int lohi = LOHI(i);
                const int lo = lohi & 0xffff, hi = lohi >> 16;
                if (j < lo || j > hi) break;
                const int c = ROWSTART(i) + (j - lo);
                const int d = (WB(c >> 4) >> ((c & 15) * 2)) & 3;
                if (d == 0) --i; else if (d == 1) --j; else { --i; --j; }
            }
        }
        out[r * n_y + a] = (float)(1.0 / (result + 1.0));
    }
#undef WD
#undef WI
#undef WB
#undef ROWSTART
#undef LOHI
#undef FL
}

#define DTW_R 32
#ifndef DTW_MINB12
#define DTW_MINB12 3
#endif
#ifndef DTW_MINB32
#define DTW_MINB32 2
#endif
#ifndef DTW_MINB20
#define DTW_MINB20 3
#endif
#define DTW_EMPTY 1

#ifdef DTW_PROBE_COUNT
__device__ unsigned long long g_dtw_counts[8][8];
extern "C" int sgnn_dtw_probe_counts(unsigned long long* out, int reset)
{
    if (out && hipMemcpyFromSymbol(out, HIP_SYMBOL(g_dtw_counts), sizeof(unsigned long long) * 64) != hipSuccess) return -1;
    if (reset) { static unsigned long long z[64]; if (hipMemcpyToSymbol(HIP_SYMBOL(g_dtw_counts), z, sizeof(z)) != hipSuccess) return -1; }
    return 0;
}
__device__ __forceinline__ unsigned long long dtw_probe_wave_sum(unsigned long long v)
{
    for (int d = 32; d >= 1; d >>= 1) v += __shfl_xor(v, d, 64);
    return v;
}
#define DTW_COUNT(LEV, WHAT, V) do { if ((threadIdx.x & 63) == 0) atomicAdd(&g_dtw_counts[(LEV) & 7][WHAT], (unsigned long long)(V)); } while (0)
#define DTW_COUNT_LANE(LEV, WHAT, V) atomicAdd(&g_dtw_counts[(LEV) & 7][WHAT], (unsigned long long)(V))
template <int P>
__device__ __forceinline__ void dtw_probe_windows(const int32_t (&lohi)[P], bool act, int lx, int lev)
{
    unsigned long long own = 0;
    for (int p = 0; p < P; ++p)
        if (lohi[p] != DTW_EMPTY) own += (unsigned long long)(((uint32_t)lohi[p] >> 16) - (lohi[p] & 0xffff) + 1) * (2 * p + 1 < lx ? 2 : 1);
    own = dtw_probe_wave_sum(own);
    const unsigned long long lanes = dtw_probe_wave_sum(act ? 1ull : 0ull);
    DTW_COUNT(lev, 0, 1); DTW_COUNT(lev, 2, own); DTW_COUNT(lev, 6, lanes);
}
#else
#define DTW_COUNT(LEV, WHAT, V) do { } while (0)
#define DTW_COUNT_LANE(LEV, WHAT, V) do { (void)(V); } while (0)
template <int P> __device__ __forceinline__ void dtw_probe_windows(const int32_t (&)[P], bool, int, int) { }
#endif

typedef unsigned short dtw_us2 __attribute__((ext_vector_type(2)));
__device__ __forceinline__ uint32_t dtw_pkmax(uint32_t a, uint32_t b) {
    const dtw_us2 m = __builtin_elementwise_max(__builtin_bit_cast(dtw_us2, a), __builtin_bit_cast(dtw_us2, b));
    return __builtin_bit_cast(uint32_t, m);
}
template <int CTRL, int ROW_MASK> __device__ __forceinline__ uint32_t dtw_dpp(uint32_t v) {
    return (uint32_t)__builtin_amdgcn_update_dpp((int)v, (int)v, CTRL, ROW_MASK, 0xf, false);
}
__device__ __forceinline__ uint32_t dtw_wave_pkmax(uint32_t v) {
    v = dtw_pkmax(v, dtw_dpp<0xb1, 0xf>(v));
    v = dtw_pkmax(v, dtw_dpp<0x4e, 0xf>(v));
    v = dtw_pkmax(v, dtw_dpp<0x124, 0xf>(v));
    v = dtw_pkmax(v, dtw_dpp<0x128, 0xf>(v));
    v = dtw_pkmax(v, dtw_dpp<0x142, 0xa>(v));
    v = dtw_pkmax(v, dtw_dpp<0x143, 0xc>(v));
    return (uint32_t)__builtin_amdgcn_readlane((int)v, 63);
}

#define FLQ(q) fl[(q) * DTW_THREADS]

template <int P>
__device__ __forceinline__ void dtw_wave_windows(int32_t* __restrict__ fl, bool act, int lx, int ly, int lxc, int lyc,
                                                 bool coarsest, int32_t (&lohi)[P], uint32_t (&hull)[P])
{
    if (coarsest) {
#pragma unroll
        for (int p = 0; p < P; ++p) lohi[p] = (act && 2 * p < lx) ? ((ly - 1) << 16) : DTW_EMPTY;
    } else {
        int prev_lo = 0;
#pragma unroll
        for (int p = 0; p < P; ++p) {
            const int ca = p - 1 < 0 ? 0 : p - 1;
            const int cb = p + 1;
            const int firstc = FLQ(ca) & 0xffff;
            const int lastc = (cb < lxc) ? (FLQ(cb < P ? cb : P - 1) >> 16) : (lyc - 1);
            int lo = 2 * (firstc - 1);
            int hi = 2 * (lastc + 1) + 1;
            if (lo < prev_lo) lo = prev_lo;
            if (lo < 0) lo = 0;
            if (hi > ly - 1) hi = ly - 1;
            int32_t v = (hi << 16) | lo;
            if (hi < lo || 2 * p >= lx || !act) v = DTW_EMPTY; else prev_lo = lo;
            lohi[p] = v;
        }
    }
#pragma unroll
    for (int p = 0; p < P; ++p) {
        const uint32_t lo = lohi[p] & 0xffff, hi = (uint32_t)lohi[p] >> 16;
        hull[p] = dtw_wave_pkmax(lohi[p] == DTW_EMPTY ? 0u : (((0x7fffu - lo) << 16) | (hi + 1)));
    }
}

#define DTW_LOAD_ROWS(INIT)                                                                                          \
    _Pragma("unroll")                                                                                                \
    for (int i = 0; i < RR; ++i) {                                                                                   \
        const int64_t ic = i < lx ? i : 0;                                    \
        xp1[i] = xcol[ic * n_x] + 1.0;                                        \
        xr[i] = xrcol[ic * n_x];                                                                                     \
        INIT;                                                                                                        \
    }

template <int P, bool LAST_ROW>
__device__ __forceinline__ uint32_t dtw_column_pairs(const uint32_t (&hull)[P], uint32_t c)
{
    uint32_t ra = P, rb1 = 0;
#pragma unroll
    for (int p = P - 1; p >= 0; --p) ra = ((hull[p] & 0xffffu) > c) ? (uint32_t)p : ra;
#pragma unroll
    for (int p = 0; p < P; ++p) rb1 = (hull[p] != 0u && (0x7fffu - (hull[p] >> 16)) <= c) ? (uint32_t)(p + 1) : rb1;
    return rb1 > ra ? ((((1u << rb1) - 1u) & ~((1u << ra) - 1u)) | (ra << 16) | (LAST_ROW ? (2u * rb1 - 1u) << 27 : 0u)) : 0u;
}

#ifdef DTW_PROBE_NO_BACKTRACK
#define DTW_BACKTRACE_CELLS(FIXED)
#else
#define DTW_BACKTRACE_CELLS(FIXED)                                                                                   \
    {                                                                                                                \
        int i = lx - 1, j = ly - 1;                                                                                  \
        int last = j;                                                                                                \
        uint32_t word = WLDS ? wl[j * DTW_THREADS] : wq[(int64_t)j * NT];                                            \
        unsigned long long bt_steps = 0;                                                  \
        while (i >= 0 && j >= 0) {                                                                                   \
            ++bt_steps;                                                                                              \
            int d;                                                                                                   \
            if constexpr (FIXED) d = (int)((word >> (2 * i)) & 3);                                                   \
            else {                                                                                                   \
                const int sh = 2 * ((int)(word >> 27) - i);                                                          \
                const uint32_t b = (word >> sh) & 3u;                                \
                if (TIE == 0) d = (b & 2u) ? 0 : ((b & 1u) ? 1 : 2);                                                 \
                else d = (b & 2u) ? 2 : ((b & 1u) ? 0 : 1);                                                          \
            }                                                                                                        \
            if (d != 1) {                                                     \
                FLQ(i) = (last << 16) | j;                                                                           \
                --i;                                                                                                 \
            }                                                                                                        \
            if (d != 0) {                                                                                            \
                --j;                                                                                                 \
                if (j >= 0) word = WLDS ? wl[j * DTW_THREADS] : wq[(int64_t)j * NT];                                 \
            }                                                                                                        \
            if (d != 1) last = j;                                             \
        }                                                                                                            \
         \
        if (i >= 0 && j < 0) FLQ(i) = (last << 16) | 0;                                                              \
        DTW_COUNT_LANE(lev, 5, bt_steps);                                                                            \
    }
#endif

template <int RR, int TIE, bool WLDS, bool FINEST>
__device__ __forceinline__ double dtw_wave_level(
    int32_t* __restrict__ fl, const double* __restrict__ xcol, const double* __restrict__ xrcol, int64_t n_x,
    const double* __restrict__ ycol, const double* __restrict__ yrcol, bool act,
    int lx, int ly, int lxc, int lyc, bool coarsest, uint32_t* __restrict__ wl, uint32_t* __restrict__ wq, int64_t NT, int lev = 0)
{
    static_assert(RR % 2 == 0 && RR <= 32, "rows come in pairs");
    constexpr int P = RR / 2;
    const double INF = __longlong_as_double(0x7ff0000000000000ll);
    int32_t lohi[P];
    uint32_t hull[P];
    dtw_wave_windows<P>(fl, act, lx, ly, lxc, lyc, coarsest, lohi, hull);
    dtw_probe_windows<P>(lohi, act, lx, lev);
    double xp1[RR], xr[RR], col[RR];
    DTW_LOAD_ROWS(col[i] = INF)
    const int lane = threadIdx.x & 63;
    uint32_t prev_am = 0;
    for (int jc = 0; jc < ly; jc += 64) {
        const uint32_t tab = dtw_column_pairs<P, false>(hull, (uint32_t)(jc + lane));
        const int jend = jc + 64 < ly ? jc + 64 : ly;
        double y_next = ycol[jc], yr_next = yrcol[jc];
        for (int j = jc; j < jend; ++j) {
            const double yp1 = y_next + 1.0, yr = yr_next;
            if (j + 1 < ly) { y_next = ycol[j + 1]; yr_next = yrcol[j + 1]; }
            const uint32_t t = (uint32_t)__builtin_amdgcn_readlane((int)tab, j - jc);
            const uint32_t am = t & 0xffffu;
            const int ra = (int)(t >> 16);
            DTW_COUNT(lev, 1, 2 * __builtin_popcount(am)); DTW_COUNT(lev, 3, 1); DTW_COUNT(lev, 4, __builtin_popcount(am));
            const bool carry = ra > 0 && ((prev_am >> (ra - 1)) & 1u);
            prev_am = am;
            uint32_t word = 0;
            double pm = INF, cd = INF, dg = INF, da = INF;
            bool in_ = false;
            double dt1_ = 0.0;
#define DTW_IN(K) { const int lo_ = lohi[(K) < P ? (K) : 0] & 0xffff, hi_ = lohi[(K) < P ? (K) : 0] >> 16; in_ = j >= lo_ && j <= hi_; }
#define DTW_COST(I) dtw_mask_cost(in_, dtw_cost_rcp(xp1[(I) < RR ? (I) : 0], xr[(I) < RR ? (I) : 0], yp1, yr))
#define DTW_CELL_A(K, UPV)                                                                                           \
            {                                                                                                        \
                constexpr int a_ = 2 * (K) < RR ? 2 * (K) : 0, b_ = 2 * (K) + 1 < RR ? 2 * (K) + 1 : 0;              \
                const double dt0_ = DTW_COST(2 * (K));                                                               \
                dt1_ = DTW_COST(2 * (K) + 1);                                                                        \
                if constexpr (FINEST) {                                                                              \
                      \
                                        \
                    const double m_ = fmin(pm, (UPV));                                                               \
                    pm = fmin(col[a_], col[b_]);                                                                     \
                    col[a_] = m_ + dt0_;                                                                             \
                } else {                                                                                             \
                    const double c_up = (UPV) + dt0_, c_left = col[a_] + dt0_, c_diag = dg + dt0_;                   \
                    const double m1_ = fmin((UPV), col[a_]);                                                         \
                    const double mv = TIE == 2 ? fmin(m1_, dg) + dt0_                                                \
                                               : fmin(fmin(c_up, c_left), c_diag);    \
                          \
                                            \
                    uint32_t best;                                                                                   \
                    if (TIE == 0) best = c_up == mv ? 0u : (c_left == mv ? 1u : 2u);         \
                    else if (TIE == 1) best = c_diag == mv ? 2u : (c_up == mv ? 0u : 1u);    \
                    else best = dg <= m1_ ? 2u : ((UPV) <= col[a_] ? 0u : 1u);            \
                    word |= best << (2 * a_);                                                                        \
                    if (TIE == 2) da = col[a_]; else cd = col[a_] + dt1_;     \
                    col[a_] = mv;                                                                                    \
                }                                                                                                    \
            }
#define DTW_CELL_B(K)                                                                                                \
            {                                                                                                        \
                constexpr int a_ = 2 * (K) < RR ? 2 * (K) : 0, b_ = 2 * (K) + 1 < RR ? 2 * (K) + 1 : 0;              \
                constexpr int c_ = 2 * (K) + 2 < RR ? 2 * (K) + 2 : b_;                                              \
                if constexpr (FINEST) {                                                                              \
                    const double m_ = fmin(pm, col[a_]);                                                             \
                    pm = fmin(col[b_], col[c_]);                                                                     \
                    col[b_] = m_ + dt1_;                                                                             \
                } else {                                                                                             \
                    const double c_up = col[a_] + dt1_, c_left = col[b_] + dt1_, c_diag = TIE == 2 ? da + dt1_ : cd; \
                    const double m1_ = fmin(col[a_], col[b_]);                                                       \
                    const double mv = TIE == 2 ? fmin(m1_, da) + dt1_ : fmin(fmin(c_up, c_left), c_diag);            \
                    uint32_t best;                                                                                   \
                    if (TIE == 0) best = c_up == mv ? 0u : (c_left == mv ? 1u : 2u);                                 \
                    else if (TIE == 1) best = c_diag == mv ? 2u : (c_up == mv ? 0u : 1u);                            \
                    else best = da <= m1_ ? 2u : (col[a_] <= col[b_] ? 0u : 1u);                                     \
                    word |= best << (2 * b_);                                                                        \
                    dg = col[b_];                                                       \
                    col[b_] = mv;                                                                                    \
                }                                                                                                    \
            }
#define DTW_PAIR(K)                                                                                                  \
            if ((K) < P && (am & (1u << (K)))) {                                                                     \
                constexpr int u_ = (2 * (K) - 1) >= 0 && (2 * (K) - 1) < RR ? (2 * (K) - 1) : 0;                     \
                DTW_IN(K)                                                                                            \
                if ((K) == 0) {                                                                                      \
                    const double diag = (j == 0) ? 0.0 : INF;                       \
                    if constexpr (FINEST) pm = fmin(diag, col[0]); else dg = diag;                                   \
                    DTW_CELL_A(K, INF)                                                                               \
                } else {                                                                                             \
                    if (ra == (K)) {                                                                                 \
                        const double diag = carry ? col[u_] : INF;                                                   \
                        if constexpr (FINEST) pm = fmin(diag, col[2 * (K) < RR ? 2 * (K) : 0]); else dg = diag;      \
                        col[u_] = INF;                                                                               \
                        asm volatile("" ::: "memory");                        \
                    }                                                                                                \
                    DTW_CELL_A(K, col[u_])                                                                           \
                }                                                                                                    \
                DTW_CELL_B(K)                                                                                        \
            }
            DTW_PAIR(0) DTW_PAIR(1) DTW_PAIR(2) DTW_PAIR(3) DTW_PAIR(4) DTW_PAIR(5) DTW_PAIR(6) DTW_PAIR(7)
            DTW_PAIR(8) DTW_PAIR(9) DTW_PAIR(10) DTW_PAIR(11) DTW_PAIR(12) DTW_PAIR(13) DTW_PAIR(14) DTW_PAIR(15)
#undef DTW_IN
#undef DTW_CELL_A
#undef DTW_CELL_B
#undef DTW_COST
#undef DTW_PAIR
            if (!FINEST) {
                if (WLDS) wl[j * DTW_THREADS] = word; else wq[(int64_t)j * NT] = word;
            }
        }
    }
    double result = 0.0;
#pragma unroll
    for (int i = 0; i < RR; ++i) if (i == lx - 1) result = col[i];
    if (FINEST || !act) return result;
    DTW_BACKTRACE_CELLS(true)
    return result;
}

__device__ __forceinline__ uint32_t dtw_shift_in(uint32_t word, uint64_t lane_mask)
{
#if defined(__gfx950__) || defined(__gfx942__) || defined(__gfx90a__)
    uint32_t out;
    asm("v_addc_co_u32_e64 %0, vcc, %1, %1, %2" : "=v"(out) : "v"(word), "s"(lane_mask) : "vcc");
    return out;
#elif defined(__HIP_DEVICE_COMPILE__)
#error "dtw_shift_in: hand-written instruction in the gfx9 family's wave64 encoding (gfx90a, gfx942, gfx950)"
#else
    return 2u * word + (uint32_t)(lane_mask & 1u);
#endif
}

template <int RR, int TIE, bool WLDS, bool ROW_MAJOR>
__device__ __forceinline__ void dtw_wave_level_2col(
    int32_t* __restrict__ fl, const double* __restrict__ xcol, const double* __restrict__ xrcol, int64_t n_x,
    const double* __restrict__ ycol, const double* __restrict__ yrcol, bool act,
    int lx, int ly, int lxc, int lyc, bool coarsest, uint32_t* __restrict__ wl, uint32_t* __restrict__ wq, int64_t NT, int lev = 0)
{
    static_assert(RR % 2 == 0 && (ROW_MAJOR ? RR <= 16 : 2 * RR <= 27),
                  "rows come in pairs; two words of bits per row, or two bits per row below the row number in a column's word");
    constexpr int P = RR / 2;
    const double INF = __longlong_as_double(0x7ff0000000000000ll);
    int32_t lohi[P];
    uint32_t hull[P];
    dtw_wave_windows<P>(fl, act, lx, ly, lxc, lyc, coarsest, lohi, hull);
    dtw_probe_windows<P>(lohi, act, lx, lev);
    double xp1[RR], xr[RR], cA[RR], cB[RR];
    [[maybe_unused]] uint32_t mA[RR], mB[RR];
    DTW_LOAD_ROWS(cA[i] = INF; cB[i] = INF; if constexpr (ROW_MAJOR) { mA[i] = 0u; mB[i] = 0u; })
    const int lane = threadIdx.x & 63;
    uint32_t prev_am = 0;
#define DTW2_IN(K) { const int lo_ = lohi[(K) < P ? (K) : 0] & 0xffff, hi_ = lohi[(K) < P ? (K) : 0] >> 16; in_ = J_ >= lo_ && J_ <= hi_; }
#define DTW2_COST(I) dtw_mask_cost(in_, dtw_cost_rcp(xp1[(I) < RR ? (I) : 0], xr[(I) < RR ? (I) : 0], yp1, yr))
#define DTW2_CELL(UPV, LEFT, DIAG, DT, OUT, ROW)                                                                     \
        {                                                                                                            \
            const double c_up = (UPV) + (DT), c_left = (LEFT) + (DT), c_diag = (DIAG) + (DT);                        \
             \
             \
             \
            const double m1_ = fmin((UPV), (LEFT));                                                                  \
            const double mv = TIE == 2 ? fmin(m1_, (DIAG)) + (DT) : fmin(fmin(c_up, c_left), c_diag);                \
            const bool first_ = TIE == 0 ? c_up == mv : (TIE == 1 ? c_diag == mv : (DIAG) <= m1_);                   \
            const bool second_ = TIE == 0 ? c_left == mv : (TIE == 1 ? c_up == mv : (UPV) <= (LEFT));                \
            if constexpr (ROW_MAJOR) {                                                                               \
                mA[ROW] = dtw_shift_in(mA[ROW], __ballot(first_));                                                   \
                mB[ROW] = dtw_shift_in(mB[ROW], __ballot(second_));                                                  \
            } else {                                                                                                 \
                word = dtw_shift_in(word, __ballot(first_));                                                         \
                word = dtw_shift_in(word, __ballot(second_));                                                        \
            }                                                                                                        \
            (OUT) = mv;                                                                                              \
        }
#define DTW2_PAIR(K, PREV, CUR)                                                                                      \
        if ((K) < P && (am & (1u << (K)))) {                                                                         \
            constexpr int a_ = 2 * (K) < RR ? 2 * (K) : 0, b_ = 2 * (K) + 1 < RR ? 2 * (K) + 1 : 0;                  \
            constexpr int u_ = (2 * (K) - 1) >= 0 && (2 * (K) - 1) < RR ? (2 * (K) - 1) : 0;                         \
            bool in_;                                                                                                \
            DTW2_IN(K)                                                                                               \
            const double dt0_ = DTW2_COST(2 * (K));                                                                  \
            const double dt1_ = DTW2_COST(2 * (K) + 1);                                                              \
            if ((K) == 0) {                                                                                          \
                const double diag0_ = (J_ == 0) ? 0.0 : INF;                        \
                DTW2_CELL(INF, PREV[a_], diag0_, dt0_, CUR[a_], a_)                                                  \
            } else {                                                                                                 \
                if (ra == (K)) {                                              \
                    CUR[u_] = INF;                                                                                   \
                    if (!carry) PREV[u_] = INF;                                                                      \
                    asm volatile("" ::: "memory");                                          \
                }                                                                                                    \
                DTW2_CELL(CUR[u_], PREV[a_], PREV[u_], dt0_, CUR[a_], a_)                                            \
            }                                                                                                        \
            DTW2_CELL(CUR[a_], PREV[b_], PREV[a_], dt1_, CUR[b_], b_)                                                \
        }
#define DTW2_COLUMN(JJ, PREV, CUR)                                                                                   \
        {                                                                                                            \
            const int J_ = (JJ);                                                                                     \
            const double yp1 = y_next + 1.0, yr = yr_next;                                                           \
            if (J_ + 1 < ly) { y_next = ycol[J_ + 1]; yr_next = yrcol[J_ + 1]; }                                     \
            const uint32_t t = (uint32_t)__builtin_amdgcn_readlane((int)tab, J_ - jc);                               \
            const uint32_t am = t & 0xffffu;                                                                         \
            const int ra = (int)((t >> 16) & 0x7ffu);                                                                \
            DTW_COUNT(lev, 1, 2 * __builtin_popcount(am)); DTW_COUNT(lev, 3, 1); DTW_COUNT(lev, 4, __builtin_popcount(am)); \
            const bool carry = ra > 0 && ((prev_am >> (ra - 1)) & 1u);                                               \
            prev_am = am;                                                                                            \
            [[maybe_unused]] uint32_t word = 0;                                                                      \
            DTW2_PAIR(0, PREV, CUR) DTW2_PAIR(1, PREV, CUR) DTW2_PAIR(2, PREV, CUR) DTW2_PAIR(3, PREV, CUR)          \
            DTW2_PAIR(4, PREV, CUR) DTW2_PAIR(5, PREV, CUR) DTW2_PAIR(6, PREV, CUR) DTW2_PAIR(7, PREV, CUR)          \
            if constexpr (!ROW_MAJOR) {                                                                              \
                word |= t & 0xf8000000u;                                                  \
                if (WLDS) wl[J_ * DTW_THREADS] = word; else wq[(int64_t)J_ * NT] = word;                             \
            }                                                                                                        \
        }
#define DTW2_CHUNK(JC, JEND)                                                                                         \
        {                                                                                                            \
            const int jc = (JC), jend = (JEND);                                                                      \
            const uint32_t tab = dtw_column_pairs<P, !ROW_MAJOR>(hull, (uint32_t)(jc + lane));                       \
            double y_next = ycol[jc], yr_next = yrcol[jc];                                                           \
            int j = jc;                                                                                              \
            for (; j + 1 < jend; j += 2) {                                                                           \
                DTW2_COLUMN(j, cB, cA)                                                                               \
                DTW2_COLUMN(j + 1, cA, cB)                                                                           \
            }                                                                                                        \
            if (j < jend) DTW2_COLUMN(j, cB, cA)                                                                     \
        }
    if constexpr (ROW_MAJOR) DTW2_CHUNK(0, ly)
    else for (int jc0 = 0; jc0 < ly; jc0 += 64) DTW2_CHUNK(jc0, jc0 + 64 < ly ? jc0 + 64 : ly)
#undef DTW2_CHUNK
#undef DTW2_IN
#undef DTW2_COST
#undef DTW2_CELL
#undef DTW2_PAIR
#undef DTW2_COLUMN
    if constexpr (!ROW_MAJOR) {
        if (!act) return;
        DTW_BACKTRACE_CELLS(false)
    } else {
#ifndef DTW_PROBE_NO_BACKTRACK
        int j = act ? ly - 1 : -1;
#pragma unroll
        for (int i = RR - 1; i >= 0; --i) {
            const uint32_t h = hull[i >> 1];
            const int uhi = (int)(h & 0xffffu) - 1, ulo = 0x7fff - (int)(h >> 16);
            if (i < lx && j >= 0) {
                const int pos = uhi - j;
                const uint32_t valid = (uhi - ulo + 1) >= 32 ? ~0u : ((1u << (uhi - ulo + 1)) - 1u);
                const uint32_t A = mA[i], B = mB[i];
                const uint32_t is_left = (TIE == 0 ? (~A & B) : (~A & ~B)) & valid;
                const uint32_t tl = (pos >= 0 && pos < 32) ? (is_left >> pos) : 0u;
                int run = __ffs((int)~tl) - 1;
                if (run < 0) run = 32;
                if (run > j) run = j;
                const int first = j - run;
                FLQ(i) = (j << 16) | first;
                const int p2 = pos + run;
                const uint32_t a2 = (p2 >= 0 && p2 < 32) ? ((A >> p2) & 1u) : 0u, b2 = (p2 >= 0 && p2 < 32) ? ((B >> p2) & 1u) : 0u;
                const bool up = TIE == 0 ? (a2 != 0u) : (a2 == 0u && b2 != 0u);
                const bool left_still = TIE == 0 ? (a2 == 0u && b2 != 0u) : (a2 == 0u && b2 == 0u);
                j = left_still ? -1 : (up ? first : first - 1);
            }
        }
#endif
    }
}
#undef FLQ
#undef DTW_LOAD_ROWS
#undef DTW_BACKTRACE_CELLS

template <int RMAX, int TIE, int MINB, bool WLDS>
__global__ __launch_bounds__(DTW_THREADS, MINB) void dtw_similarity_reg_kernel(
    const double* __restrict__ xpyr, const int32_t* __restrict__ xlen, int64_t n_x,
    const double* __restrict__ ypyr, const int32_t* __restrict__ ylen, int64_t n_y,
    float* __restrict__ out, uint32_t* __restrict__ wq, DtwLayout L, const int32_t* __restrict__ x_order,
    const int64_t* __restrict__ x_live)
{
    constexpr int RH = ((RMAX / 2) + 1) & ~1;
    __shared__ int32_t s_fl[RH * DTW_THREADS];
    extern __shared__ uint32_t s_words[];
    int32_t* fl = s_fl + threadIdx.x;
    uint32_t* wl = s_words + threadIdx.x;
    const int64_t NT = (int64_t)gridDim.x * blockDim.x;
    const int64_t tid = blockIdx.x * (int64_t)blockDim.x + threadIdx.x;
    const int lane = threadIdx.x & 63;
    const int64_t first_live = x_live ? x_live[0] : 0;
    const int64_t n_live = x_live ? x_live[1] : n_x;
    const int64_t chunks = (n_live + 63) / 64;
    const int64_t n_tasks = chunks * n_y;
    const int64_t n_waves = NT / 64;
    const int64_t wave0 = __builtin_amdgcn_readfirstlane((int)(tid >> 6));
    for (int64_t task = wave0; task < n_tasks; task += n_waves) {
        const int64_t a = task / chunks;
        const int64_t p0 = first_live + (task - a * chunks) * 64 + lane;
        const bool have = p0 < first_live + n_live;
        const int64_t pos = have ? p0 : first_live;
        const int64_t r = x_order ? x_order[pos] : pos;
        const int ly0 = ylen[a];
        const int lx0 = have ? xlen[pos] : 0;
        const bool valid = have && lx0 > 0 && ly0 > 0;
        int n_levels = 0;
        if (valid) {
            n_levels = 1;
            int lx = lx0, ly = ly0;
            while (lx >= 3 && ly >= 3) { lx >>= 1; ly >>= 1; ++n_levels; }
        }
        const int max_levels = (int)(dtw_wave_pkmax((uint32_t)n_levels) & 0xffff);
        const double* __restrict__ yp = ypyr + a * L.YL;
        double result = 0.0;
        for (int lev = max_levels - 1; lev >= 0; --lev) {
            const bool act = lev < n_levels;
            const int lx = act ? lx0 >> lev : 0, ly = ly0 >> lev;
            const int lxc = lx0 >> (lev + 1), lyc = ly0 >> (lev + 1);
            const double* xcol = xpyr + L.xoff[lev] * n_x + pos;
            const double* xrcol = xcol + L.XL * n_x;
            const double* ycol = yp + L.yoff[lev];
            const double* yrcol = ycol + L.YL * n_y;
            uint32_t* w = wq + (L.yoff[lev] - L.MY) * NT + tid;
            const bool coarsest = lev == n_levels - 1;
#ifdef DTW_PROBE_NO_FINEST
            if (lev == 0) continue;
#endif
#ifdef DTW_PROBE_NO_COARSE
            if (lev != 0) continue;
#endif
            if (lev == 0)
                result = dtw_wave_level<RMAX, TIE, WLDS, true>(fl, xcol, xrcol, n_x, ycol, yrcol, act, lx, ly, lxc, lyc,
                                                               coarsest, wl, w, NT, lev);
            else if constexpr (2 * RH <= 27) {
                if (WLDS && ly <= 32) {
                    constexpr int R2 = (((RMAX >> 2) + 1) & ~1) < 2 ? 2 : (((RMAX >> 2) + 1) & ~1);
                    constexpr int R3 = (((RMAX >> 3) + 1) & ~1) < 2 ? 2 : (((RMAX >> 3) + 1) & ~1);
                    if (lev == 1)
                        dtw_wave_level_2col<RH, TIE, WLDS, true>(fl, xcol, xrcol, n_x, ycol, yrcol, act, lx, ly, lxc, lyc, coarsest, wl, w, NT, lev);
                    else if (lev == 2)
                        dtw_wave_level_2col<R2, TIE, WLDS, true>(fl, xcol, xrcol, n_x, ycol, yrcol, act, lx, ly, lxc, lyc, coarsest, wl, w, NT, lev);
                    else
                        dtw_wave_level_2col<R3, TIE, WLDS, true>(fl, xcol, xrcol, n_x, ycol, yrcol, act, lx, ly, lxc, lyc, coarsest, wl, w, NT, lev);
                }
                else
                    dtw_wave_level_2col<RH, TIE, WLDS, false>(fl, xcol, xrcol, n_x, ycol, yrcol, act, lx, ly, lxc, lyc, coarsest, wl, w, NT, lev);
            }
            else
                dtw_wave_level<RH, TIE, WLDS, false>(fl, xcol, xrcol, n_x, ycol, yrcol, act, lx, ly, lxc, lyc, coarsest,
                                                     wl, w, NT, lev);
        }
        if (have) out[r * n_y + a] = valid ? (float)(1.0 / (result + 1.0)) : 0.f;
    }
}

__global__ void dtw_order_keys_kernel(const int64_t* __restrict__ x_ptr, const int32_t* __restrict__ x_val, int64_t n_x,
                                      int64_t* __restrict__ keys)
{
    const int64_t i = blockIdx.x * (int64_t)blockDim.x + threadIdx.x;
    if (i >= n_x) return;
    const int64_t b = x_ptr[i], len = x_ptr[i + 1] - b;
    int64_t key = (len > 0xFFF ? (int64_t)0xFFF : len) << 48;
#ifndef DTW_KEY_STEPS
#define DTW_KEY_STEPS 4.f
#endif
    auto q8 = [](float v) { const int q = (int)lrintf(DTW_KEY_STEPS * log2f(1.f + (v < 0.f ? 0.f : v))); return (int64_t)(q > 255 ? 255 : q); };
    const int64_t n2 = len / 4;
    if (n2 == 0) {
        for (int64_t f = 0; f < len; ++f) key |= q8((float)x_val[b + f]) << (40 - 8 * f);
    } else {
        const int64_t nf = n2 < 6 ? n2 : 6;
        for (int64_t f = 0; f < nf; ++f) {
            const int64_t g = b + 4 * ((f * n2) / nf);
            const float v = 0.25f * ((float)x_val[g] + (float)x_val[g + 1] + (float)x_val[g + 2] + (float)x_val[g + 3]);
            key |= q8(v) << (40 - 8 * f);
        }
    }
    keys[i] = key;
}

extern "C" int sgnn_dtw_order_keys(const int64_t* x_ptr, const int32_t* x_val, int64_t n_x, int64_t* out_keys, void* stream)
{
    if (!x_ptr || !x_val || !out_keys || n_x < 0) return SGNN_ERR_BAD_ARG;
    if (n_x == 0) return SGNN_OK;
    hipLaunchKernelGGL(dtw_order_keys_kernel, dim3((unsigned)((n_x + 255) / 256)), dim3(256), 0, (hipStream_t)stream, x_ptr,
                       x_val, n_x, out_keys);
    SGNN_CHECK_LAUNCH();
    return SGNN_OK;
}

#define DTW_ROWS_MAGIC 0x53474e4e44545752ll
#define DTW_ROWS_HEAD 8
enum { DTW_ROWS_ORDERED = 1, DTW_ROWS_NATURAL = 2 };

static inline int64_t dtw_rows_bytes(int64_t n_x, const DtwLayout& L) { return 2 * n_x * L.XL * 8 + dtw_align8(n_x * 4); }
static inline int dtw_rows_layout(int64_t max_x_len, int kernel, const int32_t* x_order) {
    return (max_x_len <= DTW_R && kernel == 0 && x_order) ? DTW_ROWS_ORDERED : DTW_ROWS_NATURAL;
}

extern "C" int64_t sgnn_dtw_rows_bytes(int64_t n_x, int64_t max_x_len) {
    if (max_x_len < 1) max_x_len = 1;
    if (n_x < 0) n_x = 0;
    return dtw_rows_bytes(n_x, dtw_layout(max_x_len, 1));
}

extern "C" int64_t sgnn_dtw_rows_header_words(void) { return DTW_ROWS_HEAD; }

extern "C" int64_t sgnn_dtw_rows_workspace_bytes(int64_t n_x, int64_t max_x_len, int64_t n_y, int64_t max_y_len) {
    return sgnn_dtw_workspace_bytes(n_x, max_x_len, n_y, max_y_len) - sgnn_dtw_rows_bytes(n_x, max_x_len);
}

static void dtw_prepare_rows(const int64_t* x_ptr, const int32_t* x_val, int64_t n_x, int64_t max_x_len, const DtwLayout& L,
                             int layout, const int32_t* x_order, char* rows, hipStream_t st)
{
    double* xpyr = (double*)rows;
    int32_t* xlen = (int32_t*)(rows + 2 * n_x * L.XL * 8);
    dtw_launch_pyramid(x_ptr, x_val, n_x, max_x_len, L.XL, 1, xpyr, xpyr + n_x * L.XL, xlen,
                       layout == DTW_ROWS_ORDERED ? x_order : (const int32_t*)nullptr, st);
}

extern "C" int sgnn_dtw_prepare_rows(const int64_t* x_ptr, const int32_t* x_val, int64_t n_x, int64_t max_x_len, int kernel,
                                     const int32_t* x_order, void* rows, int64_t rows_bytes, int64_t* header, void* stream)
{
    if (!x_ptr || !x_val || !rows || !header || n_x < 0 || kernel < 0 || kernel > 1) return SGNN_ERR_BAD_ARG;
    if (max_x_len < 1) max_x_len = 1;
    if (max_x_len > 32767) return SGNN_ERR_SET_TOO_LARGE;
    const DtwLayout L = dtw_layout(max_x_len, 1);
    if (rows_bytes < dtw_rows_bytes(n_x, L)) return SGNN_ERR_BAD_ARG;
    const int layout = dtw_rows_layout(max_x_len, kernel, x_order);
    header[0] = 0;
    if (n_x > 0) {
        dtw_prepare_rows(x_ptr, x_val, n_x, max_x_len, L, layout, x_order, (char*)rows, (hipStream_t)stream);
        SGNN_CHECK_LAUNCH();
    }
    header[1] = layout; header[2] = n_x; header[3] = max_x_len; header[4] = (int64_t)(intptr_t)rows; header[5] = rows_bytes;
    header[6] = header[7] = 0;
    header[0] = DTW_ROWS_MAGIC;
    return SGNN_OK;
}

static int dtw_run_rows(const char* rows, int64_t n_x, int64_t max_x_len,
                        const int64_t* y_ptr, const int32_t* y_val, int64_t n_y, int64_t max_y_len,
                        int tie_order, int kernel, const int32_t* x_order, const int64_t* x_live, float* out, void* workspace,
                        hipStream_t st)
{
    const DtwLayout L = dtw_layout(max_x_len, max_y_len);
    char* w = (char*)workspace;
    const int64_t scratch = dtw_scratch_bytes(L);
    double* wd = (double*)w;
    int32_t* wi = (int32_t*)(w + DTW_NT * L.n_dbl * 8);
    uint32_t* wb = (uint32_t*)(w + DTW_NT * (L.n_dbl * 8 + dtw_align8(L.n_i32 * 4)));
    uint32_t* wq = (uint32_t*)w;           w += scratch;
    double* ypyr = (double*)w;             w += 2 * n_y * L.YL * 8;
    int32_t* ylen = (int32_t*)w;
    const double* xpyr = (const double*)rows;
    const int32_t* xlen = (const int32_t*)(rows + 2 * n_x * L.XL * 8);
    const bool use_reg = max_x_len <= DTW_R && kernel == 0;
    dtw_launch_pyramid(y_ptr, y_val, n_y, max_y_len, L.YL, 0, ypyr, ypyr + n_y * L.YL, ylen, (const int32_t*)nullptr, st);
    SGNN_CHECK_LAUNCH();
    if (use_reg) {
        const int64_t words = max_y_len >> 1;
        const bool wlds = dtw_words_in_lds(max_y_len);
        size_t dyn = wlds ? (size_t)((words > 0 ? words : 1) * DTW_THREADS * 4) : 0;
#ifdef DTW_PROBE_LDS_PAD
        static const long lds_pad = getenv("SGNN_DTW_LDS_PAD") ? atol(getenv("SGNN_DTW_LDS_PAD")) : 0;
        if (lds_pad > 0) dyn += (size_t)(lds_pad < (long)(48 * 1024 - (long)dyn) ? lds_pad : (48 * 1024 > (long)dyn ? 48 * 1024 - (long)dyn : 0));
#endif
#define DTW_LAUNCH2(RMAX, TIE, MINB, WL) \
        hipLaunchKernelGGL((dtw_similarity_reg_kernel<RMAX, TIE, MINB, WL>), dim3(DTW_REG_BLOCKS), dim3(DTW_THREADS), dyn, st, \
                           xpyr, xlen, n_x, ypyr, ylen, n_y, out, wq, L, x_order, x_live)
#define DTW_LAUNCH(RMAX, TIE, MINB) do { if (wlds) DTW_LAUNCH2(RMAX, TIE, MINB, true); else DTW_LAUNCH2(RMAX, TIE, MINB, false); } while (0)
#define DTW_LAUNCH_T(RMAX, MINB) do { if (tie_order == 0) DTW_LAUNCH(RMAX, 0, MINB); else if (tie_order == 1) DTW_LAUNCH(RMAX, 1, MINB); else DTW_LAUNCH(RMAX, 2, MINB); } while (0)
        if (max_x_len <= 12) DTW_LAUNCH_T(12, DTW_MINB12);
        else if (max_x_len <= 20) DTW_LAUNCH_T(20, DTW_MINB20);
        else DTW_LAUNCH_T(32, DTW_MINB32);
#undef DTW_LAUNCH_T
#undef DTW_LAUNCH2
#undef DTW_LAUNCH
    } else {
        hipLaunchKernelGGL(dtw_similarity_kernel, dim3(DTW_BLOCKS), dim3(DTW_THREADS), 0, st, xpyr, xlen, n_x, ypyr,
                           ylen, n_y, tie_order, out, wd, wi, wb, L);
    }
    SGNN_CHECK_LAUNCH();
    return SGNN_OK;
}

static int dtw_run(const int64_t* x_ptr, const int32_t* x_val, int64_t n_x, int64_t max_x_len,
                   const int64_t* y_ptr, const int32_t* y_val, int64_t n_y, int64_t max_y_len,
                   int tie_order, int kernel, const int32_t* x_order, const int64_t* x_live, float* out, void* workspace,
                   int64_t workspace_bytes, void* stream)
{
    if (!x_ptr || !x_val || !y_ptr || !y_val || !out || !workspace || n_x < 0 || n_y < 0) return SGNN_ERR_BAD_ARG;
    if (tie_order < 0 || tie_order > 2 || kernel < 0 || kernel > 1) return SGNN_ERR_BAD_ARG;
    if (max_x_len < 1) max_x_len = 1;
    if (max_y_len < 1) max_y_len = 1;
    if (max_x_len > 32767 || max_y_len > 32767) return SGNN_ERR_SET_TOO_LARGE;
    if (workspace_bytes < sgnn_dtw_workspace_bytes(n_x, max_x_len, n_y, max_y_len)) return SGNN_ERR_BAD_ARG;
    if (n_x * n_y == 0) return SGNN_OK;
    const DtwLayout L = dtw_layout(max_x_len, max_y_len);
    char* rows = (char*)workspace + sgnn_dtw_rows_workspace_bytes(n_x, max_x_len, n_y, max_y_len);
    dtw_prepare_rows(x_ptr, x_val, n_x, max_x_len, L, dtw_rows_layout(max_x_len, kernel, x_order), x_order, rows, (hipStream_t)stream);
    SGNN_CHECK_LAUNCH();
    return dtw_run_rows(rows, n_x, max_x_len, y_ptr, y_val, n_y, max_y_len, tie_order, kernel, x_order, x_live, out, workspace,
                        (hipStream_t)stream);
}

static int dtw_run_prepared(const int64_t* header, int64_t n_x, int64_t max_x_len,
                            const int64_t* y_ptr, const int32_t* y_val, int64_t n_y, int64_t max_y_len,
                            int tie_order, int kernel, const int32_t* x_order, const int64_t* x_live, float* out, void* workspace,
                            int64_t workspace_bytes, void* stream)
{
    if (!header || !y_ptr || !y_val || !out || !workspace || n_x < 0 || n_y < 0) return SGNN_ERR_BAD_ARG;
    if (tie_order < 0 || tie_order > 2 || kernel < 0 || kernel > 1) return SGNN_ERR_BAD_ARG;
    if (max_x_len < 1) max_x_len = 1;
    if (max_y_len < 1) max_y_len = 1;
    if (max_x_len > 32767 || max_y_len > 32767) return SGNN_ERR_SET_TOO_LARGE;
    if (header[0] != DTW_ROWS_MAGIC || header[2] != n_x || header[3] != max_x_len || !header[4]) return SGNN_ERR_BAD_ARG;
    if (header[1] != dtw_rows_layout(max_x_len, kernel, x_order)) return SGNN_ERR_BAD_ARG;
    if (header[5] < dtw_rows_bytes(n_x, dtw_layout(max_x_len, 1))) return SGNN_ERR_BAD_ARG;
    if (workspace_bytes < sgnn_dtw_rows_workspace_bytes(n_x, max_x_len, n_y, max_y_len)) return SGNN_ERR_BAD_ARG;
    if (n_x * n_y == 0) return SGNN_OK;
    return dtw_run_rows((const char*)(intptr_t)header[4], n_x, max_x_len, y_ptr, y_val, n_y, max_y_len, tie_order, kernel, x_order,
                        x_live, out, workspace, (hipStream_t)stream);
}

extern "C" int sgnn_dtw_similarity(const int64_t* x_ptr, const int32_t* x_val, int64_t n_x, int64_t max_x_len,
                                   const int64_t* y_ptr, const int32_t* y_val, int64_t n_y, int64_t max_y_len,
                                   int tie_order, int kernel, const int32_t* x_order, float* out, void* workspace,
                                   int64_t workspace_bytes, void* stream)
{
    return dtw_run(x_ptr, x_val, n_x, max_x_len, y_ptr, y_val, n_y, max_y_len, tie_order, kernel, x_order, nullptr, out, workspace,
                   workspace_bytes, stream);
}

extern "C" int sgnn_dtw_similarity_live(const int64_t* x_ptr, const int32_t* x_val, int64_t n_x, int64_t max_x_len,
                                        const int64_t* y_ptr, const int32_t* y_val, int64_t n_y, int64_t max_y_len,
                                        int tie_order, int kernel, const int32_t* x_order, const int64_t* x_live_range,
                                        float* out, void* workspace, int64_t workspace_bytes, void* stream)
{
    if (x_live_range && !x_order) return SGNN_ERR_BAD_ARG;
    return dtw_run(x_ptr, x_val, n_x, max_x_len, y_ptr, y_val, n_y, max_y_len, tie_order, kernel, x_order, x_live_range, out,
                   workspace, workspace_bytes, stream);
}

extern "C" int sgnn_dtw_similarity_rows(const int64_t* rows_header, int64_t n_x, int64_t max_x_len,
                                        const int64_t* y_ptr, const int32_t* y_val, int64_t n_y, int64_t max_y_len,
                                        int tie_order, int kernel, const int32_t* x_order, float* out, void* workspace,
                                        int64_t workspace_bytes, void* stream)
{
    return dtw_run_prepared(rows_header, n_x, max_x_len, y_ptr, y_val, n_y, max_y_len, tie_order, kernel, x_order, nullptr, out,
                            workspace, workspace_bytes, stream);
}

extern "C" int sgnn_dtw_similarity_rows_live(const int64_t* rows_header, int64_t n_x, int64_t max_x_len,
                                             const int64_t* y_ptr, const int32_t* y_val, int64_t n_y, int64_t max_y_len,
                                             int tie_order, int kernel, const int32_t* x_order, const int64_t* x_live_range,
                                             float* out, void* workspace, int64_t workspace_bytes, void* stream)
{
    if (x_live_range && !x_order) return SGNN_ERR_BAD_ARG;
    return dtw_run_prepared(rows_header, n_x, max_x_len, y_ptr, y_val, n_y, max_y_len, tie_order, kernel, x_order, x_live_range,
                            out, workspace, workspace_bytes, stream);
}

SGNN_DEFINE_WARM(dtw)
```

subgnn_amd/csrc/dtw_cost.h:

```cpp
#pragma once
#include <hip/hip_runtime.h>

__device__ static inline double dtw_cost(double a, double b) {
    const double mx = a > b ? a : b, mn = a > b ? b : a;
    return (mx + 1.0) / (mn + 1.0) - 1.0;
}

__device__ __forceinline__ double dtw_cost_rcp(double a1, double ra, double b1, double rb) {
    const double mx = fmax(a1, b1), mn = fmin(a1, b1), r = fmax(ra, rb);
    const double q0 = __dmul_rn(mx, r);
    const double q = __fma_rn(__fma_rn(-q0, mn, mx), r, q0);
    return __dadd_rn(q, -1.0);
}
```

Baseline: 7.943 million subgraphs/s.

## Use atomic work-stealing and occupancy-sized grid for DTW register kernel

Replaces the fixed 8192-block grid-stride DTW register kernel with a grid sized to resident occupancy (capped by task count). Each wave draws tasks dynamically from a global atomic counter stored just before ylen in the workspace, and a memset resets that counter before every launch. The pyramid now stores values pre-offset by +1, and the window mask is folded into a bias add (-1 or a huge value), which removes a +1.0 add and a select per cell. The change adds atomic traffic, a memset, a cached occupancy query and workspace layout changes, and shifts the rows-layout enum values.

Result: slower. 6.940 million subgraphs/s (-12.6%).

```diff
diff --git a/include/subgnn_hip.h b/include/subgnn_hip.h
--- a/include/subgnn_hip.h
+++ b/include/subgnn_hip.h
@@ -226,6 +226,7 @@
                         const int64_t* y_ptr, const int32_t* y_val, int64_t n_y, int64_t max_y_len,
                         int tie_order, int kernel, const int32_t* x_order, float* out, void* workspace,
                         int64_t workspace_bytes, void* stream);
+int64_t sgnn_dtw_reg_launch_waves(int64_t n_x, int64_t max_x_len, int64_t n_y, int64_t max_y_len, int tie_order);
 int sgnn_dtw_similarity_live(const int64_t* x_ptr, const int32_t* x_val, int64_t n_x, int64_t max_x_len,
                              const int64_t* y_ptr, const int32_t* y_val, int64_t n_y, int64_t max_y_len,
                              int tie_order, int kernel, const int32_t* x_order, const int64_t* x_live_range, float* out,
diff --git a/subgnn_amd/_lib.py b/subgnn_amd/_lib.py
--- a/subgnn_amd/_lib.py
+++ b/subgnn_amd/_lib.py
@@ -101,6 +101,7 @@
     'sgnn_bfs_hops': (c_int, [c_ptr, c_ptr, c_i64, c_i64, c_ptr, c_i64, c_int, c_int, c_int, c_ptr, c_ptr, c_i64, c_ptr]),
     'sgnn_min_hops_to_sets': (c_int, [c_ptr, c_i64, c_i64, c_int, c_ptr, c_ptr, c_i64, c_ptr, c_ptr]),
     'sgnn_dtw_workspace_bytes': (c_i64, [c_i64, c_i64, c_i64, c_i64]),
+    'sgnn_dtw_reg_launch_waves': (c_i64, [c_i64, c_i64, c_i64, c_i64, c_int]),
     'sgnn_dtw_similarity': (c_int, [c_ptr, c_ptr, c_i64, c_i64, c_ptr, c_ptr, c_i64, c_i64, c_int, c_int, c_ptr, c_ptr, c_ptr,
                                     c_i64, c_ptr]),
     'sgnn_dtw_order_keys': (c_int, [c_ptr, c_ptr, c_i64, c_ptr, c_ptr]),
diff --git a/subgnn_amd/build.py b/subgnn_amd/build.py
--- a/subgnn_amd/build.py
+++ b/subgnn_amd/build.py
@@ -8,7 +8,8 @@
 LIB = os.path.join(LIBDIR, 'libsubgnn_hip.so')
 SOURCES = ['lib.hip', 'degree_sequence.hip', 'graph_sets.hip', 'samplers.hip', 'similarity.hip', 'dtw.hip', 'dtw_exact.hip', 'embed.hip', 'mpn.hip', 'attention.hip', 'lstm.hip', 'probe.hip', 'scatter.hip', 'update.hip', 'optim.hip', 'readout.hip', 'loss.hip', 'head.hip', 'node_emb.hip', 'subgraph_props.hip', 'neighbors.hip', 'occlusion.hip', 'insertion.hip', 'seeded_sets.hip', 'kmeans.hip']
 ARCH = 'gfx950'
-EXTRA_FLAGS = {'dtw.hip': ['-fno-honor-nans', '-mllvm', '-disable-promote-alloca-to-vector'],
+EXTRA_FLAGS = {'dtw.hip': ['-fno-honor-nans', '-mllvm', '-disable-promote-alloca-to-vector',
+                           '-mllvm', '-amdgpu-atomic-optimizer-strategy=None'],
                'dtw_exact.hip': ['-fno-honor-nans', '-mllvm', '-disable-promote-alloca-to-vector']}
 HEADERS = [os.path.join(CSRC, 'common.h'), os.path.join(CSRC, 'dtw_cost.h'), os.path.join(CSRC, 'id_table.h'), os.path.join(CSRC, 'topk_order.h'), os.path.join(HERE, '..', 'include', 'subgnn_hip.h')]
 
diff --git a/subgnn_amd/csrc/dtw.hip b/subgnn_amd/csrc/dtw.hip
--- a/subgnn_amd/csrc/dtw.hip
+++ b/subgnn_amd/csrc/dtw.hip
@@ -2,16 +2,14 @@
 #include "dtw_cost.h"
 #include <type_traits>
 #include <cstdlib>
+#include <mutex>
 
 #define DTW_THREADS 256
 #ifndef DTW_BLOCKS
 #define DTW_BLOCKS (256 * 2)
 #endif
 #define DTW_NT ((int64_t)DTW_THREADS * DTW_BLOCKS)
-#ifndef DTW_REG_BLOCKS
-#define DTW_REG_BLOCKS (256 * 32)
-#endif
-#define DTW_REG_NT ((int64_t)DTW_THREADS * DTW_REG_BLOCKS)
+#define DTW_REG_MAX_BLOCKS (256 * 32)
 #define DTW_MAX_LEVELS 16
 
 struct DtwLayout {
@@ -42,19 +40,27 @@
 static inline int64_t dtw_align8(int64_t b) { return (b + 7) / 8 * 8; }
 
 static inline bool dtw_words_in_lds(int64_t max_y_len) { return (max_y_len >> 1) * DTW_THREADS * 4 <= 48 * 1024; }
-static inline int64_t dtw_scratch_bytes(const DtwLayout& L) {
+static inline int64_t dtw_reg_task_blocks(int64_t n_x, int64_t n_y) {
+    const int64_t tasks = (n_x + 63) / 64 * n_y, per_block = DTW_THREADS / 64;
+    const int64_t b = (tasks + per_block - 1) / per_block;
+    return b < 1 ? 1 : (b > DTW_REG_MAX_BLOCKS ? DTW_REG_MAX_BLOCKS : b);
+}
+static inline int64_t dtw_scratch_bytes(const DtwLayout& L, int64_t n_x, int64_t n_y) {
     const int64_t lane = L.n_dbl * 8 + dtw_align8(L.n_i32 * 4) + dtw_align8(L.n_dir * 4);
     int64_t scratch = DTW_NT * lane;
-    const int64_t reg = dtw_words_in_lds(L.MY) ? 0 : dtw_align8(DTW_REG_NT * (L.YL - L.MY) * 4);
+    const int64_t reg = dtw_words_in_lds(L.MY) ? 0 : dtw_align8(dtw_reg_task_blocks(n_x, n_y) * DTW_THREADS * (L.YL - L.MY) * 4);
     return reg > scratch ? reg : scratch;
 }
 
 extern "C" int64_t sgnn_dtw_workspace_bytes(int64_t n_x, int64_t max_x_len, int64_t n_y, int64_t max_y_len) {
     if (max_x_len < 1) max_x_len = 1;
     if (max_y_len < 1) max_y_len = 1;
+    if (n_x < 0) n_x = 0;
+    if (n_y < 0) n_y = 0;
     const DtwLayout L = dtw_layout(max_x_len, max_y_len);
-    return dtw_scratch_bytes(L)
-         + 2 * (n_x * L.XL * 8 + n_y * L.YL * 8) + dtw_align8(n_x * 4) + dtw_align8(n_y * 4);
+    return dtw_scratch_bytes(L, n_x, n_y)
+         + 2 * (n_x * L.XL * 8 + n_y * L.YL * 8) + dtw_align8(n_x * 4) + dtw_align8(n_y * 4)
+         + 8;
 }
 
 __global__ void dtw_pyramid_kernel(const int64_t* __restrict__ ptr, const int32_t* __restrict__ val, int64_t n,
@@ -69,7 +75,7 @@
         len_out[s] = len;
 #define PYI(e) (transposed ? (int64_t)(e) * n + s : s * PL + (e))
 #define PY(e) out[PYI(e)]
-        for (int i = 0; i < len; ++i) { const double v = (double)val[b + i]; PY(i) = v; rec[PYI(i)] = 1.0 / (v + 1.0); }
+        for (int i = 0; i < len; ++i) { const double v = (double)val[b + i] + 1.0; PY(i) = v; rec[PYI(i)] = 1.0 / v; }
         int64_t off = 0;
         int k = 0;
         while (len >= 2 && k + 1 < DTW_MAX_LEVELS) {
@@ -78,7 +84,7 @@
             for (int i = 0; i < nlen; ++i) {
                 const double v = (PY(off + 2 * i) + PY(off + 2 * i + 1)) / 2.0;
                 PY(noff + i) = v;
-                rec[PYI(noff + i)] = 1.0 / (v + 1.0);
+                rec[PYI(noff + i)] = 1.0 / v;
             }
             off = noff; len = nlen; ++k;
         }
@@ -103,10 +109,10 @@
     if (lane == 0) len_out[s] = len;
 #define PYI(e) (transposed ? (int64_t)(e) * n + s : s * PL + (e))
     for (int i = lane; i < len; i += 64) {
-        const double v = (double)val[b + i];
+        const double v = (double)val[b + i] + 1.0;
         buf[i] = v;
         out[PYI(i)] = v;
-        rec[PYI(i)] = 1.0 / (v + 1.0);
+        rec[PYI(i)] = 1.0 / v;
     }
     int64_t off = 0;
     int k = 0;
@@ -120,7 +126,7 @@
             const double v = (buf[off + 2 * i] + buf[off + 2 * i + 1]) / 2.0;
             buf[noff + i] = v;
             out[PYI(noff + i)] = v;
-            rec[PYI(noff + i)] = 1.0 / (v + 1.0);
+            rec[PYI(noff + i)] = 1.0 / v;
         }
         off = noff; len = nlen; ++k;
     }
@@ -141,9 +147,18 @@
                            rec, len_out, order);
 }
 
-__device__ __forceinline__ double dtw_mask_cost(bool in, double dt) {
-    return __hiloint2double(in ? __double2hiint(dt) : 0x7fe00000, __double2loint(dt));
-}
+__device__ __forceinline__ uint32_t dtw_opaque(uint32_t v) {
+#if defined(__HIP_DEVICE_COMPILE__)
+    asm("" : "+v"(v));
+#endif
+    return v;
+}
+__device__ __forceinline__ double dtw_window_bias(bool in, uint32_t m1hi, double bias) {
+    return __hiloint2double((int)(in ? m1hi : 0x7fe00000u), __double2loint(bias));
+}
+#define DTW_BIAS_INIT                                                         \
+    const uint32_t m1hi = dtw_opaque(0xbff00000u);                                                                   \
+    double bias = __hiloint2double((int)m1hi, (int)dtw_opaque(0u));
 
 __global__ __launch_bounds__(DTW_THREADS) void dtw_similarity_kernel(
     const double* __restrict__ xpyr, const int32_t* __restrict__ xlen, int64_t n_x,
@@ -362,7 +377,7 @@
     _Pragma("unroll")                                                                                                \
     for (int i = 0; i < RR; ++i) {                                                                                   \
         const int64_t ic = i < lx ? i : 0;                                    \
-        xp1[i] = xcol[ic * n_x] + 1.0;                                        \
+        xp1[i] = xcol[ic * n_x];                                              \
         xr[i] = xrcol[ic * n_x];                                                                                     \
         INIT;                                                                                                        \
     }
@@ -413,11 +428,18 @@
     }
 #endif
 
+__device__ __forceinline__ uint32_t dtw_draw_task(uint32_t* next_task, int lane) {
+    uint32_t drawn = 0;
+    if (lane == 0) drawn = __hip_atomic_fetch_add(next_task, 1u, __ATOMIC_RELAXED, __HIP_MEMORY_SCOPE_AGENT);
+    return drawn;
+}
+
 template <int RR, int TIE, bool WLDS, bool FINEST>
 __device__ __forceinline__ double dtw_wave_level(
     int32_t* __restrict__ fl, const double* __restrict__ xcol, const double* __restrict__ xrcol, int64_t n_x,
     const double* __restrict__ ycol, const double* __restrict__ yrcol, bool act,
-    int lx, int ly, int lxc, int lyc, bool coarsest, uint32_t* __restrict__ wl, uint32_t* __restrict__ wq, int64_t NT, int lev = 0)
+    int lx, int ly, int lxc, int lyc, bool coarsest, uint32_t* __restrict__ wl, uint32_t* __restrict__ wq, int64_t NT, int lev = 0,
+    uint32_t* next_task = nullptr, uint32_t* drawn = nullptr)
 {
     static_assert(RR % 2 == 0 && RR <= 32, "rows come in pairs");
     constexpr int P = RR / 2;
@@ -429,13 +451,15 @@
     double xp1[RR], xr[RR], col[RR];
     DTW_LOAD_ROWS(col[i] = INF)
     const int lane = threadIdx.x & 63;
+    if constexpr (FINEST) { if (next_task) *drawn = dtw_draw_task(next_task, lane); }
     uint32_t prev_am = 0;
+    DTW_BIAS_INIT
     for (int jc = 0; jc < ly; jc += 64) {
         const uint32_t tab = dtw_column_pairs<P, false>(hull, (uint32_t)(jc + lane));
         const int jend = jc + 64 < ly ? jc + 64 : ly;
         double y_next = ycol[jc], yr_next = yrcol[jc];
         for (int j = jc; j < jend; ++j) {
-            const double yp1 = y_next + 1.0, yr = yr_next;
+            const double yp1 = y_next, yr = yr_next;
             if (j + 1 < ly) { y_next = ycol[j + 1]; yr_next = yrcol[j + 1]; }
             const uint32_t t = (uint32_t)__builtin_amdgcn_readlane((int)tab, j - jc);
             const uint32_t am = t & 0xffffu;
@@ -445,10 +469,9 @@
             prev_am = am;
             uint32_t word = 0;
             double pm = INF, cd = INF, dg = INF, da = INF;
-            bool in_ = false;
             double dt1_ = 0.0;
-#define DTW_IN(K) { const int lo_ = lohi[(K) < P ? (K) : 0] & 0xffff, hi_ = lohi[(K) < P ? (K) : 0] >> 16; in_ = j >= lo_ && j <= hi_; }
-#define DTW_COST(I) dtw_mask_cost(in_, dtw_cost_rcp(xp1[(I) < RR ? (I) : 0], xr[(I) < RR ? (I) : 0], yp1, yr))
+#define DTW_IN(K) { const int lo_ = lohi[(K) < P ? (K) : 0] & 0xffff, hi_ = lohi[(K) < P ? (K) : 0] >> 16; bias = dtw_window_bias(j >= lo_ && j <= hi_, m1hi, bias); }
+#define DTW_COST(I) __dadd_rn(dtw_quot_rcp(xp1[(I) < RR ? (I) : 0], xr[(I) < RR ? (I) : 0], yp1, yr), bias)
 #define DTW_CELL_A(K, UPV)                                                                                           \
             {                                                                                                        \
                 constexpr int a_ = 2 * (K) < RR ? 2 * (K) : 0, b_ = 2 * (K) + 1 < RR ? 2 * (K) + 1 : 0;              \
@@ -568,8 +591,9 @@
     DTW_LOAD_ROWS(cA[i] = INF; cB[i] = INF; if constexpr (ROW_MAJOR) { mA[i] = 0u; mB[i] = 0u; })
     const int lane = threadIdx.x & 63;
     uint32_t prev_am = 0;
-#define DTW2_IN(K) { const int lo_ = lohi[(K) < P ? (K) : 0] & 0xffff, hi_ = lohi[(K) < P ? (K) : 0] >> 16; in_ = J_ >= lo_ && J_ <= hi_; }
-#define DTW2_COST(I) dtw_mask_cost(in_, dtw_cost_rcp(xp1[(I) < RR ? (I) : 0], xr[(I) < RR ? (I) : 0], yp1, yr))
+    DTW_BIAS_INIT
+#define DTW2_IN(K) { const int lo_ = lohi[(K) < P ? (K) : 0] & 0xffff, hi_ = lohi[(K) < P ? (K) : 0] >> 16; bias = dtw_window_bias(J_ >= lo_ && J_ <= hi_, m1hi, bias); }
+#define DTW2_COST(I) __dadd_rn(dtw_quot_rcp(xp1[(I) < RR ? (I) : 0], xr[(I) < RR ? (I) : 0], yp1, yr), bias)
 #define DTW2_CELL(UPV, LEFT, DIAG, DT, OUT, ROW)                                                                     \
         {                                                                                                            \
             const double c_up = (UPV) + (DT), c_left = (LEFT) + (DT), c_diag = (DIAG) + (DT);                        \
@@ -593,7 +617,6 @@
         if ((K) < P && (am & (1u << (K)))) {                                                                         \
             constexpr int a_ = 2 * (K) < RR ? 2 * (K) : 0, b_ = 2 * (K) + 1 < RR ? 2 * (K) + 1 : 0;                  \
             constexpr int u_ = (2 * (K) - 1) >= 0 && (2 * (K) - 1) < RR ? (2 * (K) - 1) : 0;                         \
-            bool in_;                                                                                                \
             DTW2_IN(K)                                                                                               \
             const double dt0_ = DTW2_COST(2 * (K));                                                                  \
             const double dt1_ = DTW2_COST(2 * (K) + 1);                                                              \
@@ -613,7 +636,7 @@
 #define DTW2_COLUMN(JJ, PREV, CUR)                                                                                   \
         {                                                                                                            \
             const int J_ = (JJ);                                                                                     \
-            const double yp1 = y_next + 1.0, yr = yr_next;                                                           \
+            const double yp1 = y_next, yr = yr_next;                                                                 \
             if (J_ + 1 < ly) { y_next = ycol[J_ + 1]; yr_next = yrcol[J_ + 1]; }                                     \
             const uint32_t t = (uint32_t)__builtin_amdgcn_readlane((int)tab, J_ - jc);                               \
             const uint32_t am = t & 0xffffu;                                                                         \
@@ -687,7 +710,7 @@
 template <int RMAX, int TIE, int MINB, bool WLDS>
 __global__ __launch_bounds__(DTW_THREADS, MINB) void dtw_similarity_reg_kernel(
     const double* __restrict__ xpyr, const int32_t* __restrict__ xlen, int64_t n_x,
-    const double* __restrict__ ypyr, const int32_t* __restrict__ ylen, int64_t n_y,
+    const double* __restrict__ ypyr, int32_t* __restrict__ ylen, int64_t n_y,
     float* __restrict__ out, uint32_t* __restrict__ wq, DtwLayout L, const int32_t* __restrict__ x_order,
     const int64_t* __restrict__ x_live)
 {
@@ -696,18 +719,20 @@
     extern __shared__ uint32_t s_words[];
     int32_t* fl = s_fl + threadIdx.x;
     uint32_t* wl = s_words + threadIdx.x;
-    const int64_t NT = (int64_t)gridDim.x * blockDim.x;
-    const int64_t tid = blockIdx.x * (int64_t)blockDim.x + threadIdx.x;
+    const int64_t NT = (int64_t)gridDim.x * DTW_THREADS;
+    const int64_t tid = blockIdx.x * (int64_t)DTW_THREADS + threadIdx.x;
     const int lane = threadIdx.x & 63;
     const int64_t first_live = x_live ? x_live[0] : 0;
     const int64_t n_live = x_live ? x_live[1] : n_x;
-    const int64_t chunks = (n_live + 63) / 64;
-    const int64_t n_tasks = chunks * n_y;
-    const int64_t n_waves = NT / 64;
-    const int64_t wave0 = __builtin_amdgcn_readfirstlane((int)(tid >> 6));
-    for (int64_t task = wave0; task < n_tasks; task += n_waves) {
-        const int64_t a = task / chunks;
-        const int64_t p0 = first_live + (task - a * chunks) * 64 + lane;
+    const uint32_t chunks = (uint32_t)((uint64_t)(n_live + 63) >> 6);
+    const uint32_t n_tasks = chunks * (uint32_t)n_y;
+    uint32_t* next_task = (uint32_t*)ylen - 2;
+    uint32_t drawn = dtw_draw_task(next_task, lane);
+    for (;;) {
+        const uint32_t task = (uint32_t)__builtin_amdgcn_readfirstlane((int)drawn);
+        if (task >= n_tasks) break;
+        const uint32_t a = task / chunks;
+        const int64_t p0 = first_live + (int64_t)(task - a * chunks) * 64 + lane;
         const bool have = p0 < first_live + n_live;
         const int64_t pos = have ? p0 : first_live;
         const int64_t r = x_order ? x_order[pos] : pos;
@@ -721,8 +746,9 @@
             while (lx >= 3 && ly >= 3) { lx >>= 1; ly >>= 1; ++n_levels; }
         }
         const int max_levels = (int)(dtw_wave_pkmax((uint32_t)n_levels) & 0xffff);
-        const double* __restrict__ yp = ypyr + a * L.YL;
+        const double* __restrict__ yp = ypyr + (int64_t)a * L.YL;
         double result = 0.0;
+        if (max_levels == 0) drawn = dtw_draw_task(next_task, lane);
         for (int lev = max_levels - 1; lev >= 0; --lev) {
             const bool act = lev < n_levels;
             const int lx = act ? lx0 >> lev : 0, ly = ly0 >> lev;
@@ -741,7 +767,7 @@
 #endif
             if (lev == 0)
                 result = dtw_wave_level<RMAX, TIE, WLDS, true>(fl, xcol, xrcol, n_x, ycol, yrcol, act, lx, ly, lxc, lyc,
-                                                               coarsest, wl, w, NT, lev);
+                                                               coarsest, wl, w, NT, lev, next_task, &drawn);
             else if constexpr (2 * RH <= 27) {
                 if (WLDS && ly <= 32) {
                     constexpr int R2 = (((RMAX >> 2) + 1) & ~1) < 2 ? 2 : (((RMAX >> 2) + 1) & ~1);
@@ -760,7 +786,7 @@
                 dtw_wave_level<RH, TIE, WLDS, false>(fl, xcol, xrcol, n_x, ycol, yrcol, act, lx, ly, lxc, lyc, coarsest,
                                                      wl, w, NT, lev);
         }
-        if (have) out[r * n_y + a] = valid ? (float)(1.0 / (result + 1.0)) : 0.f;
+        if (have) out[r * n_y + (int64_t)a] = valid ? (float)(1.0 / (result + 1.0)) : 0.f;
     }
 }
 
@@ -801,7 +827,7 @@
 
 #define DTW_ROWS_MAGIC 0x53474e4e44545752ll
 #define DTW_ROWS_HEAD 8
-enum { DTW_ROWS_ORDERED = 1, DTW_ROWS_NATURAL = 2 };
+enum { DTW_ROWS_ORDERED = 3, DTW_ROWS_NATURAL = 4 };
 
 static inline int64_t dtw_rows_bytes(int64_t n_x, const DtwLayout& L) { return 2 * n_x * L.XL * 8 + dtw_align8(n_x * 4); }
 static inline int dtw_rows_layout(int64_t max_x_len, int kernel, const int32_t* x_order) {
@@ -849,6 +875,77 @@
     return SGNN_OK;
 }
 
+template <int RMAX, int TIE, int MINB, bool WL>
+static int64_t dtw_reg_resident_blocks(size_t dyn)
+{
+    static std::mutex mu;
+    static int c_dev = -1;
+    static size_t c_dyn = 0;
+    static int64_t c_blocks = 0;
+    int dev = 0;
+    if (hipGetDevice(&dev) != hipSuccess) return -1;
+    std::lock_guard<std::mutex> guard(mu);
+    if (dev == c_dev && dyn == c_dyn) return c_blocks;
+    int per_cu = 0, cus = 0;
+    if (hipOccupancyMaxActiveBlocksPerMultiprocessor(&per_cu, dtw_similarity_reg_kernel<RMAX, TIE, MINB, WL>, DTW_THREADS, dyn) != hipSuccess
+        || per_cu < 1) return -1;
+    if (hipDeviceGetAttribute(&cus, hipDeviceAttributeMultiprocessorCount, dev) != hipSuccess || cus < 1) return -1;
+    c_dev = dev; c_dyn = dyn; c_blocks = (int64_t)per_cu * cus;
+    return c_blocks;
+}
+
+struct DtwRegCall {
+    const double* xpyr; const int32_t* xlen; int64_t n_x; const double* ypyr;
+    int32_t* ylen;
+    int64_t n_y; float* out; uint32_t* wq; DtwLayout L; const int32_t* x_order; const int64_t* x_live;
+    size_t dyn; hipStream_t st;
+    bool query_only;
+    int64_t blocks;
+};
+
+template <int RMAX, int TIE, int MINB, bool WL>
+static int dtw_reg_launch(DtwRegCall& c)
+{
+    const int64_t resident = dtw_reg_resident_blocks<RMAX, TIE, MINB, WL>(c.dyn), by_tasks = dtw_reg_task_blocks(c.n_x, c.n_y);
+    if (resident < 1) return SGNN_ERR_LAUNCH;
+    c.blocks = resident < by_tasks ? resident : by_tasks;
+    if (c.query_only) return SGNN_OK;
+    if (hipMemsetAsync((unsigned long long*)c.ylen - 1, 0, sizeof(unsigned long long), c.st) != hipSuccess) return SGNN_ERR_LAUNCH;
+    hipLaunchKernelGGL((dtw_similarity_reg_kernel<RMAX, TIE, MINB, WL>), dim3((unsigned)c.blocks), dim3(DTW_THREADS), c.dyn, c.st,
+                       c.xpyr, c.xlen, c.n_x, c.ypyr, c.ylen, c.n_y, c.out, c.wq, c.L, c.x_order, c.x_live);
+    return SGNN_OK;
+}
+
+static int dtw_reg_dispatch(int64_t max_x_len, int64_t max_y_len, int tie_order, DtwRegCall& c)
+{
+    const int64_t words = max_y_len >> 1;
+    const bool wlds = dtw_words_in_lds(max_y_len);
+    size_t dyn = wlds ? (size_t)((words > 0 ? words : 1) * DTW_THREADS * 4) : 0;
+#ifdef DTW_PROBE_LDS_PAD
+    static const long lds_pad = getenv("SGNN_DTW_LDS_PAD") ? atol(getenv("SGNN_DTW_LDS_PAD")) : 0;
+    if (lds_pad > 0) dyn += (size_t)(lds_pad < (long)(48 * 1024 - (long)dyn) ? lds_pad : (48 * 1024 > (long)dyn ? 48 * 1024 - (long)dyn : 0));
+#endif
+    c.dyn = dyn;
+#define DTW_LAUNCH(RMAX, TIE, MINB) (wlds ? dtw_reg_launch<RMAX, TIE, MINB, true>(c) : dtw_reg_launch<RMAX, TIE, MINB, false>(c))
+#define DTW_LAUNCH_T(RMAX, MINB) (tie_order == 0 ? DTW_LAUNCH(RMAX, 0, MINB) : tie_order == 1 ? DTW_LAUNCH(RMAX, 1, MINB) : DTW_LAUNCH(RMAX, 2, MINB))
+    if (max_x_len <= 12) return DTW_LAUNCH_T(12, DTW_MINB12);
+    if (max_x_len <= 20) return DTW_LAUNCH_T(20, DTW_MINB20);
+    return DTW_LAUNCH_T(32, DTW_MINB32);
+#undef DTW_LAUNCH_T
+#undef DTW_LAUNCH
+}
+
+extern "C" int64_t sgnn_dtw_reg_launch_waves(int64_t n_x, int64_t max_x_len, int64_t n_y, int64_t max_y_len, int tie_order)
+{
+    if (max_x_len < 1) max_x_len = 1;
+    if (max_y_len < 1) max_y_len = 1;
+    if (n_x < 0 || n_y < 0 || max_x_len > DTW_R || max_y_len > 32767 || tie_order < 0 || tie_order > 2) return -1;
+    DtwRegCall c = {};
+    c.n_x = n_x; c.n_y = n_y; c.query_only = true;
+    if (dtw_reg_dispatch(max_x_len, max_y_len, tie_order, c) != SGNN_OK) return -1;
+    return c.blocks * (DTW_THREADS / 64);
+}
+
 static int dtw_run_rows(const char* rows, int64_t n_x, int64_t max_x_len,
                         const int64_t* y_ptr, const int32_t* y_val, int64_t n_y, int64_t max_y_len,
                         int tie_order, int kernel, const int32_t* x_order, const int64_t* x_live, float* out, void* workspace,
@@ -856,37 +953,24 @@
 {
     const DtwLayout L = dtw_layout(max_x_len, max_y_len);
     char* w = (char*)workspace;
-    const int64_t scratch = dtw_scratch_bytes(L);
+    const int64_t scratch = dtw_scratch_bytes(L, n_x, n_y);
     double* wd = (double*)w;
     int32_t* wi = (int32_t*)(w + DTW_NT * L.n_dbl * 8);
     uint32_t* wb = (uint32_t*)(w + DTW_NT * (L.n_dbl * 8 + dtw_align8(L.n_i32 * 4)));
     uint32_t* wq = (uint32_t*)w;           w += scratch;
     double* ypyr = (double*)w;             w += 2 * n_y * L.YL * 8;
+    w += 8;
     int32_t* ylen = (int32_t*)w;
     const double* xpyr = (const double*)rows;
     const int32_t* xlen = (const int32_t*)(rows + 2 * n_x * L.XL * 8);
     const bool use_reg = max_x_len <= DTW_R && kernel == 0;
+    if (use_reg && (n_x + 63) / 64 > ((int64_t)0x7fffffff - DTW_REG_MAX_BLOCKS * (DTW_THREADS / 64)) / n_y) return SGNN_ERR_SET_TOO_LARGE;
     dtw_launch_pyramid(y_ptr, y_val, n_y, max_y_len, L.YL, 0, ypyr, ypyr + n_y * L.YL, ylen, (const int32_t*)nullptr, st);
     SGNN_CHECK_LAUNCH();
     if (use_reg) {
-        const int64_t words = max_y_len >> 1;
-        const bool wlds = dtw_words_in_lds(max_y_len);
-        size_t dyn = wlds ? (size_t)((words > 0 ? words : 1) * DTW_THREADS * 4) : 0;
-#ifdef DTW_PROBE_LDS_PAD
-        static const long lds_pad = getenv("SGNN_DTW_LDS_PAD") ? atol(getenv("SGNN_DTW_LDS_PAD")) : 0;
-        if (lds_pad > 0) dyn += (size_t)(lds_pad < (long)(48 * 1024 - (long)dyn) ? lds_pad : (48 * 1024 > (long)dyn ? 48 * 1024 - (long)dyn : 0));
-#endif
-#define DTW_LAUNCH2(RMAX, TIE, MINB, WL) \
-        hipLaunchKernelGGL((dtw_similarity_reg_kernel<RMAX, TIE, MINB, WL>), dim3(DTW_REG_BLOCKS), dim3(DTW_THREADS), dyn, st, \
-                           xpyr, xlen, n_x, ypyr, ylen, n_y, out, wq, L, x_order, x_live)
-#define DTW_LAUNCH(RMAX, TIE, MINB) do { if (wlds) DTW_LAUNCH2(RMAX, TIE, MINB, true); else DTW_LAUNCH2(RMAX, TIE, MINB, false); } while (0)
-#define DTW_LAUNCH_T(RMAX, MINB) do { if (tie_order == 0) DTW_LAUNCH(RMAX, 0, MINB); else if (tie_order == 1) DTW_LAUNCH(RMAX, 1, MINB); else DTW_LAUNCH(RMAX, 2, MINB); } while (0)
-        if (max_x_len <= 12) DTW_LAUNCH_T(12, DTW_MINB12);
-        else if (max_x_len <= 20) DTW_LAUNCH_T(20, DTW_MINB20);
-        else DTW_LAUNCH_T(32, DTW_MINB32);
-#undef DTW_LAUNCH_T
-#undef DTW_LAUNCH2
-#undef DTW_LAUNCH
+        DtwRegCall c = {xpyr, xlen, n_x, ypyr, ylen, n_y, out, wq, L, x_order, x_live, 0, st, false, 0};
+        const int rc = dtw_reg_dispatch(max_x_len, max_y_len, tie_order, c);
+        if (rc != SGNN_OK) { sgnn_set_last_error(hipGetLastError()); return rc; }
     } else {
         hipLaunchKernelGGL(dtw_similarity_kernel, dim3(DTW_BLOCKS), dim3(DTW_THREADS), 0, st, xpyr, xlen, n_x, ypyr,
                            ylen, n_y, tie_order, out, wd, wi, wb, L);
diff --git a/subgnn_amd/csrc/dtw_cost.h b/subgnn_amd/csrc/dtw_cost.h
--- a/subgnn_amd/csrc/dtw_cost.h
+++ b/subgnn_amd/csrc/dtw_cost.h
@@ -1,14 +1,17 @@
 #pragma once
 #include <hip/hip_runtime.h>
 
-__device__ static inline double dtw_cost(double a, double b) {
-    const double mx = a > b ? a : b, mn = a > b ? b : a;
-    return (mx + 1.0) / (mn + 1.0) - 1.0;
+__device__ static inline double dtw_cost(double a1, double b1) {
+    const double mx = a1 > b1 ? a1 : b1, mn = a1 > b1 ? b1 : a1;
+    return mx / mn - 1.0;
+}
+
+__device__ __forceinline__ double dtw_quot_rcp(double a1, double ra, double b1, double rb) {
+    const double mx = fmax(a1, b1), mn = fmin(a1, b1), r = fmax(ra, rb);
+    const double q0 = __dmul_rn(mx, r);
+    return __fma_rn(__fma_rn(-q0, mn, mx), r, q0);
 }
 
 __device__ __forceinline__ double dtw_cost_rcp(double a1, double ra, double b1, double rb) {
-    const double mx = fmax(a1, b1), mn = fmin(a1, b1), r = fmax(ra, rb);
-    const double q0 = __dmul_rn(mx, r);
-    const double q = __fma_rn(__fma_rn(-q0, mn, mx), r, q0);
-    return __dadd_rn(q, -1.0);
+    return __dadd_rn(dtw_quot_rcp(a1, ra, b1, rb), -1.0);
 }
```
